# vvvvvw/Sentinel

Measured on AMD Instinct MI355X. Metric: decided entries/sec (whole node) at 1M resources; % of HBM roofline, higher is better.
Workload: dtype int64/f64

## Files before the change

sentinel_amd/csrc/engine.cpp:

```cpp
#include <hip/hip_runtime.h>

#include <algorithm>
#include <array>
#include <chrono>
#include <cmath>
#include <cstdint>
#include <cstdio>
#include <cstdlib>
#include <cstring>
#include <functional>
#include <map>
#include <set>
#include <string>
#include <unordered_map>
#include <vector>

#include "../../include/sentinel_gpu.h"
#include "authority.h"
#include "dev_types.h"
#include "pkeys.h"
#include "pmap.h"

namespace sg {
hipError_t launch_rs_first(const sg_event* ev, uint64_t n, uint32_t max_res, uint64_t gbase, const uint8_t* ring,
                           uint64_t ring_mask, int32_t max_rt, SEv* rec_o, uint32_t* keys, uint32_t* vals,
                           uint32_t* ghist, uint32_t nblocks, uint32_t* bflags, int64_t* t0_out, uint32_t* prio,
                           uint64_t* key_ring, const uint32_t* comp, const sg_event_ext* ext, const sg_arg* args,
                           uint64_t n_args, uint32_t max_ctx, const AuthDesc* auth, const uint32_t* auth_ids,
                           hipStream_t st);
hipError_t launch_radix_hist(const uint32_t* keys, uint64_t n, int shift, uint32_t* ghist, uint32_t nblocks,
                             hipStream_t st);
hipError_t launch_radix_hist_n(const uint32_t* keys, uint64_t n, const uint32_t* ndev, int shift, uint32_t* ghist,
                               uint32_t nblocks, hipStream_t st);
hipError_t launch_radix_scatter_n(const uint32_t* kin, const uint32_t* vin, uint64_t n, const uint32_t* ndev, int shift,
                                  const uint32_t* goff, uint32_t nblocks, uint32_t* kout, uint32_t* vout, hipStream_t st);
hipError_t launch_radix_scatter_x(const uint32_t* kin, const uint32_t* vin, uint64_t n, const uint32_t* ndev,
                                  const uint32_t* tcnt, const uint32_t* dbase, int shift, const uint32_t* goff,
                                  uint32_t nblocks, uint32_t* kout, uint32_t* vout, uint32_t* pos_of, hipStream_t st);
hipError_t launch_grp_first(const sg_event* ev, uint64_t n, uint32_t max_res, uint64_t gbase, uint64_t ring_mask,
                            uint32_t* bflags, int64_t* t0_out, uint32_t* prio, uint64_t* key_ring, const uint32_t* comp,
                            const sg_event_ext* ext, const sg_arg* args, uint64_t n_args, uint32_t max_ctx,
                            const AuthDesc* auth, const uint32_t* auth_ids,
                            const uint16_t* hot_tab, uint32_t nhot, uint32_t nblocks, uint32_t* words,
                            uint32_t* hot_hist, uint32_t* ckeys, uint32_t* cvals, uint32_t* ccnt, uint32_t* chist,
                            hipStream_t st);
hipError_t launch_hot_scan(uint32_t* C, uint32_t nblocks, uint32_t nhot, uint32_t* part, uint32_t* hb, uint32_t* total,
                           hipStream_t st);
hipError_t launch_hot_bmax(const sg_event* ev, uint32_t nblocks, const uint32_t* P, uint32_t nhot, const uint32_t* hb,
                           uint32_t* edges, uint32_t* bmax, hipStream_t st);
hipError_t launch_grp_records(const sg_event* ev, uint64_t n, uint64_t gbase, uint64_t ring_mask, int32_t max_rt,
                              const uint32_t* words, const uint32_t* P, uint32_t nhot, uint32_t nblocks,
                              const uint32_t* hb, SEv* recs, uint32_t* svals, uint32_t* prev,
                              uint32_t* nprev, uint32_t* bst, uint32_t* bflags, const sg_event_ext* ext,
                              const sg_arg* args, uint32_t max_ctx, Link* link, uint32_t epoch,
                              const uint32_t* need_hot, const uint32_t* need_blk, hipStream_t st);
hipError_t launch_hot_segs(const uint32_t* hb, uint32_t nhot, const uint32_t* hot_list, Seg* segs, uint32_t* out,
                           hipStream_t st);
hipError_t launch_hot_build(const Seg* segs, const uint32_t* mp, uint32_t mb, uint32_t min_len, uint32_t max_res, uint16_t* hot_tab,
                            uint32_t* hot_list, uint32_t nhot_old, uint32_t* hot_n, hipStream_t st);
hipError_t launch_cold_n(uint64_t n, const uint32_t* hot_total, uint32_t* out, hipStream_t st);
hipError_t launch_cold_small(const uint32_t* kin, const uint32_t* vin, const uint32_t* cnt, const uint32_t* dbase,
                             uint32_t* kout, uint32_t* vout, uint32_t* words, hipStream_t st);
uint32_t hot_max();
hipError_t launch_seg_cold(const uint32_t* keys, uint64_t n, const uint32_t* lo, const uint32_t* sbase, uint32_t* flag,
                           uint32_t* pos, Seg* segs, hipStream_t st,
                           hipError_t (*scan)(const uint32_t*, uint32_t*, uint64_t, uint32_t*, uint32_t*, hipStream_t),
                           uint32_t* part, uint32_t* ccount, uint32_t* nseg);
hipError_t launch_block_sums(const SEv* recs, uint64_t n, uint32_t* bst, Link* link, uint32_t epoch, uint32_t* bflags,
                             const uint32_t* skeys, const uint32_t* lo, const uint32_t* need_blk, hipStream_t st);
hipError_t launch_radix_scatter(const uint32_t* kin, const uint32_t* vin, uint64_t n, int shift, const uint32_t* goff,
                                uint32_t nblocks, uint32_t* kout, uint32_t* vout, uint32_t* pos_of, hipStream_t st);
uint32_t radix_tile();
hipError_t launch_scan(const uint32_t*, uint32_t*, uint64_t, uint32_t*, uint32_t*, hipStream_t);
hipError_t launch_snapshot(Bkt*, NodeInfo*, uint32_t, int64_t, int32_t, uint32_t*, uint32_t*, uint32_t*, uint32_t*,
                           sg_metric_node*, uint64_t, hipStream_t);
hipError_t launch_init_state(Bkt* sec, Bkt* minb, NodeInfo* info, int64_t* borrow, uint32_t nres, hipStream_t st);
hipError_t launch_set_flags(NodeInfo* info, const uint64_t* upd, uint32_t n, hipStream_t st);
hipError_t launch_region_copy(const uint64_t* src, uint64_t* dst, const uint64_t* tri, uint32_t n, hipStream_t st);
hipError_t launch_seg(const uint32_t* keys, uint64_t n, uint32_t* flag, uint32_t* pos, Seg* segs, hipStream_t st,
                      hipError_t (*scan)(const uint32_t*, uint32_t*, uint64_t, uint32_t*, uint32_t*, hipStream_t),
                      uint32_t* part, uint32_t* nseg);
hipError_t launch_seg_bin(Seg* segs, const uint32_t* mp, uint32_t mb, uint64_t n, const Prog* prog, const uint32_t* prio,
                          uint32_t lane_max, uint32_t j1_max, uint32_t j4_max, uint32_t force_lane, uint32_t* blkcnt,
                          uint32_t pq_ok, uint32_t pq_wide, uint32_t* aux, uint32_t* ashort, uint64_t* along,
                          uint64_t* amulti, uint32_t* mixc, uint32_t* mix, uint32_t mix_cap, uint32_t* mixlen,
                          uint32_t mix_wide, uint32_t head_min, const uint16_t* hot_tab, uint32_t nhot,
                          const uint32_t* nhotseg, uint32_t* need_hot, uint32_t* need_blk, const uint32_t* bmax,
                          uint32_t skip_min, uint32_t* nmark, hipStream_t st);
hipError_t launch_aux(const SEv* recs, const Seg* segs, const uint32_t* aux, const uint32_t* ashort,
                      const uint64_t* along, uint64_t* apiece, const uint64_t* amulti, const DevState& S, const DevCfg& cfg,
                      int64_t t0, const uint32_t* dec, AuxAcc* pool, uint32_t pool_cap, uint32_t* pool_n, uint64_t* meta,
                      uint32_t* bflags, hipStream_t st);
hipError_t launch_aux_cold(const SEv* recs, const Seg* segs, const uint32_t* aux, const uint32_t* ashort, const DevState& S,
                           const DevCfg& cfg, int64_t t0, const uint32_t* dec, uint32_t* bflags, hipStream_t st);
hipError_t launch_pq(int wide, const SEv* recs, const sg_event* ev, const uint32_t* vals, const Seg* segs,
                     const uint32_t* order, uint32_t m, const DevState& S, const DevCfg& cfg, int64_t t0, uint32_t* dec,
                     uint32_t* bflags, hipStream_t st);
hipError_t launch_pm_grow(const Seg* segs, const uint32_t* mp, uint32_t mb, const DevState& S, unsigned long long* pool_next,
                          uint64_t pool_nb, uint32_t* bflags, uint4* mv, uint32_t* nmv, uint32_t mcap, uint32_t epoch,
                          uint32_t nm, PBucket* b2, PData* d2, uint32_t* sz, uint32_t* off, uint32_t* part,
                          hipError_t (*scan)(const uint32_t*, uint32_t*, uint64_t, uint32_t*, uint32_t*, hipStream_t),
                          hipStream_t st);
hipError_t launch_pm_compact(PMap* pm, uint32_t n, const PBucket* ob, const PData* od, PBucket* nbk, PData* nd,
                             uint32_t* sz, uint32_t* off, uint32_t* part, unsigned long long* pool_next,
                             hipError_t (*scan)(const uint32_t*, uint32_t*, uint64_t, uint32_t*, uint32_t*, hipStream_t),
                             hipStream_t st);
hipError_t launch_pm_grow_ids(const uint32_t* ids, uint32_t n, const DevState& S, unsigned long long* pool_next,
                              uint64_t pool_nb, uint32_t* bflags, hipStream_t st);
hipError_t launch_pv_a(SEv* recs, const uint32_t* vals, Seg* segs, const uint32_t* list, uint32_t m,
                       const DevState& S, const DevCfg& cfg, uint32_t* dec, PvSeg* pv, PvBuf B, uint32_t cap,
                       uint32_t* tot, uint32_t* hist, uint32_t* part, hipStream_t st,
                       hipError_t (*radix_hist)(const uint32_t*, uint64_t, const uint32_t*, int, uint32_t*, uint32_t, hipStream_t),
                       hipError_t (*radix_scatter)(const uint32_t*, const uint32_t*, uint64_t, const uint32_t*, int,
                                                   const uint32_t*, uint32_t, uint32_t*, uint32_t*, hipStream_t),
                       hipError_t (*scan)(const uint32_t*, uint32_t*, uint64_t, uint32_t*, uint32_t*, hipStream_t),
                       uint32_t tile, uint32_t* rest, uint32_t grant_all);
hipError_t launch_pv_b(SEv* recs, Seg* segs, const uint32_t* list, uint32_t m, const DevState& S, int64_t t0,
                       uint32_t* dec, uint32_t* bflags, PvSeg* pv, PvBuf B, uint32_t cap, uint32_t* tot, uint32_t* part,
                       uint32_t jumps, hipStream_t st,
                       hipError_t (*scan)(const uint32_t*, uint32_t*, uint64_t, uint32_t*, uint32_t*, hipStream_t),
                       uint32_t* rest);
hipError_t launch_pvt(SEv* recs, const sg_event* ev, const uint32_t* vals, Seg* segs, const uint32_t* list, uint32_t m,
                      const DevState& S, const DevCfg& cfg, uint32_t* dec, uint32_t* bflags, PvSeg* pv, PvBuf B,
                      uint32_t cap, uint32_t* tot, uint32_t* hist, uint32_t* part, hipStream_t st,
                      hipError_t (*radix_hist)(const uint32_t*, uint64_t, const uint32_t*, int, uint32_t*, uint32_t, hipStream_t),
                      hipError_t (*radix_scatter)(const uint32_t*, const uint32_t*, uint64_t, const uint32_t*, int,
                                                      const uint32_t*, uint32_t, uint32_t*, uint32_t*, hipStream_t),
                      hipError_t (*scan)(const uint32_t*, uint32_t*, uint64_t, uint32_t*, uint32_t*, hipStream_t),
                      uint32_t tile, uint32_t* rest);
hipError_t launch_pq_mix(int post, SEv* recs, const sg_event* ev, const uint32_t* vals, const Seg* segs,
                         const uint32_t* list, uint32_t n_narrow, uint64_t wide_off, uint32_t n_wide, const DevState& S,
                         const DevCfg& cfg, int64_t t0, uint32_t* dec, uint32_t* bflags, hipStream_t st,
                         const uint32_t* rest, const uint32_t* rest_n);
hipError_t launch_seg_order(Seg* segs, const uint32_t* mp, uint32_t mb, const uint32_t* off, uint32_t* order,
                            uint32_t* bin_off, hipStream_t st);
hipError_t launch_gather(const SEv* rec_o, const uint32_t* vals, const uint32_t* skeys, uint64_t n,
                         const uint32_t* pos_of, SEv* recs, uint32_t* prev, uint32_t* nprev, Link* link, uint32_t* bst,
                         uint32_t epoch, uint32_t* bflags, hipStream_t st);
hipError_t launch_fill(const Span* spans, const uint32_t* nspan, uint32_t cap, const SEv* recs, const Prog* prog,
                       const DRule* rules, uint32_t* dec, hipStream_t st);
hipError_t launch_resolve(const uint32_t* prev, uint32_t np, const uint8_t* ring, SEv* recs, const uint32_t* vals,
                          const sg_event_ext* ext, hipStream_t st);
hipError_t launch_post_w(const uint32_t* words, const uint32_t* P, uint32_t nhot, const uint32_t* dec, uint64_t n,
                         uint64_t gbase, uint8_t* ring, uint64_t ring_mask, uint32_t* out, hipStream_t st);
hipError_t launch_post(const uint32_t* pos_of, const uint32_t* dec, uint64_t n, uint64_t gbase, uint8_t* ring,
                       uint64_t ring_mask, uint32_t* out, hipStream_t st);
hipError_t launch_chain(const SEv* recs, const uint32_t* vals, const Seg* segs, uint32_t m, NodeInfo* info,
                        uint32_t grant_all, uint32_t* ncand, uint64_t* cand, const sg_event* ev, const Prog* prog,
                        const sg_event_ext* ext, uint32_t max_ctx, hipStream_t st);
hipError_t launch_tiny(const sg_event* ev, uint32_t n, const DevState& S, const DevCfg& cfg, uint32_t max_res,
                       uint32_t* prio_w, const uint32_t* comp, uint64_t n_args, uint32_t grant_all,
                       unsigned long long* pool_next, uint64_t pool_nb, uint32_t epoch, SEv* recs, uint32_t* vals,
                       uint32_t* dec, Seg* segs, uint32_t* bflags, uint32_t* out, hipStream_t st);
uint32_t tiny_max();
hipError_t launch_decide_bin(int bin, const SEv* recs, const sg_event* ev, const uint32_t* vals, const Seg* segs,
                             const uint32_t* order, uint32_t m, const DevState& S, const DevCfg& cfg, int64_t t0,
                             uint32_t* dec, uint32_t* bflags, hipStream_t st);
hipError_t launch_tok_classify(const sg_token_req* req, uint64_t n, const CSlot* tab, uint32_t mask, uint32_t* fidx,
                               sg_token_result* res, uint32_t* flags, uint32_t* nskeys, uint32_t* nsvals, uint32_t nns,
                               hipStream_t st);
hipError_t launch_tok_limiter_ns(const sg_token_req* req, uint64_t n, const uint32_t* sk, const uint32_t* sv,
                                 const uint32_t* fidx, uint32_t nflows, NsLimiter* lims, const double* limits,
                                 uint32_t nns, uint32_t* keys, uint32_t* vals, sg_token_result* res, uint32_t* bflag,
                                 uint32_t* bidx, uint32_t* bstart, uint32_t* kpass, uint32_t* part, uint32_t* small,
                                 uint32_t* nsb,
                                 hipError_t (*scan)(const uint32_t*, uint32_t*, uint64_t, uint32_t*, uint32_t*, hipStream_t),
                                 hipStream_t st);
hipError_t launch_tok_limiter_par(const sg_token_req* req, uint64_t n, const uint32_t* fidx, uint32_t nflows,
                                  NsLimiter* lim, double allowed, uint32_t* keys, uint32_t* vals, sg_token_result* res,
                                  uint32_t* bflag, uint32_t* cflag, uint32_t* bidx, uint32_t* cexcl, uint32_t* bstart,
                                  uint32_t* kpass, uint32_t* part, uint32_t* small,
                                  hipError_t (*scan)(const uint32_t*, uint32_t*, uint64_t, uint32_t*, uint32_t*, hipStream_t),
                                  hipStream_t st);
hipError_t launch_tok_limiter(const sg_token_req* req, uint64_t n, const uint32_t* fidx, uint32_t nflows,
                              NsLimiter* lim, double allowed, uint32_t* keys, uint32_t* vals, sg_token_result* res,
                              hipStream_t st);
hipError_t launch_tok_flow(const uint32_t* skeys, const uint32_t* svals, uint64_t n, const sg_token_req* req,
                           CFlow* flows, uint32_t nflows, CBkt* bkts, double exceed, double max_occ_ratio,
                           sg_token_result* res, uint32_t* bounds, uint32_t light, uint32_t wide, hipStream_t st,
                           hipStream_t hs, hipEvent_t fork, hipEvent_t join);
hipError_t launch_ptok_flow(const uint32_t* skeys, const uint32_t* svals, uint64_t n, const sg_param_token_req* req,
                            const uint64_t* values, PFlow* flows, uint32_t nflows, const PHot* hot, PVal* tab,
                            uint32_t mask, sg_token_result* res, uint32_t* flags, hipStream_t st);
hipError_t launch_keysweep(const PMap* pmap, uint32_t nm, const PBucket* pbkt, uint64_t pool_nb, const uint64_t* pbm,
                           uint64_t bm_words, const uint64_t* key_ring, uint64_t ring_n, const PVal* pvtab,
                           uint64_t pv_n, const uint64_t* tkey, const uint32_t* tidx, uint32_t tmask, uint32_t* marks,
                           hipEvent_t* ev, hipStream_t st);
}

using namespace sg;

namespace {

thread_local std::string g_err;

int fail(int code, const std::string& msg) {
    g_err = msg;
    return code;
}

#define HIPCHK(x)                                                                                        \
    do {                                                                                                 \
        hipError_t _e = (x);                                                                             \
        if (_e != hipSuccess) return fail(SG_EDEVICE, std::string(#x ": ") + hipGetErrorString(_e));    \
    } while (0)

int32_t j_string_hash(const char* s) {
    if (!s) return 0;
    uint32_t h = 0;
    const unsigned char* p = (const unsigned char*)s;
    while (*p) {
        uint32_t cp;
        if (*p < 0x80) cp = *p++;
        else if ((*p & 0xE0) == 0xC0 && p[1]) { cp = ((p[0] & 0x1Fu) << 6) | (p[1] & 0x3Fu); p += 2; }
        else if ((*p & 0xF0) == 0xE0 && p[1] && p[2]) { cp = ((p[0] & 0x0Fu) << 12) | ((p[1] & 0x3Fu) << 6) | (p[2] & 0x3Fu); p += 3; }
        else if (p[1] && p[2] && p[3]) { cp = ((p[0] & 0x07u) << 18) | ((p[1] & 0x3Fu) << 12) | ((p[2] & 0x3Fu) << 6) | (p[3] & 0x3Fu); p += 4; }
// ... 168 lines not shown
              r.cluster_window_interval_ms % r.cluster_sample_count == 0))
            return false;
        if (r.cluster_flow_id <= 0) return false;
    }
    return true;
}
ParamR make_param(const sg_param_rule& s, const std::function<uint64_t(const char*, const char*)>& key) {
    ParamR p;
    p.r = s;
    p.res = sv(s.resource);
    p.la = la_norm(s.limit_app);
    for (int i = 0; i < s.n_items; ++i) {
        const sg_param_item& it = s.items[i];
        ParamItemR q;
        q.has_obj = it.object != nullptr;
        q.obj = sv(it.object);
        q.has_ct = it.class_type != nullptr;
        q.ct = sv(it.class_type);
        q.count = it.count;
        q.has_count = it.has_count;
        p.items.push_back(q);
        if (!it.object || !it.has_count || it.count < 0) continue;
        uint64_t k = key(it.object, it.class_type);
        bool found = false;
        for (auto& h : p.hot) if (h.first == k) { h.second = it.count; found = true; }
        if (!found) p.hot.push_back({k, it.count});
    }
    int32_t h = abstract_hash(s.resource, s.limit_app && !blank(s.limit_app) ? s.limit_app : "default");
    h = h31(h, s.grade);
    h = h31(h, s.has_param_idx ? s.param_idx : 0);
    h = h31(h, j_double_hash(s.count));
    h = h31(h, s.control_behavior);
    h = h31(h, s.max_queueing_time_ms);
    h = h31(h, s.burst_count);
    h = h31(h, long_hash(s.duration_in_sec));
    int32_t lh = 1;
    for (auto& q : p.items) {
        int32_t e = q.has_obj ? j_string_hash(q.obj.c_str()) : 0;
        e = h31(e, q.has_count ? q.count : 0);
        e = h31(e, q.has_ct ? j_string_hash(q.ct.c_str()) : 0);
        lh = h31(lh, e);
    }
    h = h31(h, lh);
    h = h31(h, s.cluster_mode ? 1 : 0);
    int32_t ch = 0;
    if (s.cluster_mode || s.cluster_flow_id)
        ch = cluster_hash(s.cluster_flow_id, s.cluster_threshold_type, s.cluster_fallback_to_local, 0,
                          s.cluster_sample_count, s.cluster_window_interval_ms, false);
    p.hash = h31(h, ch);
    char buf[512];
    std::snprintf(buf, sizeof(buf), "%d|%016llx|%d|%d|%d|%lld|%d|%d:%d|", s.grade, (unsigned long long)dbl_bits(s.count),
                  s.control_behavior, s.max_queueing_time_ms, s.burst_count, (long long)s.duration_in_sec,
                  s.cluster_mode ? 1 : 0, s.has_param_idx, s.has_param_idx ? s.param_idx : 0);
    std::string k = std::string(buf) + p.res + "\x01" + p.la + "\x01";
    for (auto& q : p.items) {
        std::snprintf(buf, sizeof(buf), "[%d%d%d:%d]", q.has_obj, q.has_ct, q.has_count, q.has_count ? q.count : 0);
        k += buf + q.obj + "\x02" + q.ct + "\x03";
    }
    if (s.cluster_mode || s.cluster_flow_id) {
        std::snprintf(buf, sizeof(buf), "C%lld|%d|%d|%d|%d", (long long)s.cluster_flow_id, s.cluster_threshold_type,
                      s.cluster_fallback_to_local ? 1 : 0, s.cluster_sample_count, s.cluster_window_interval_ms);
        k += buf;
    }
    p.eqkey = k;
    return p;
}

template <class T> void dfree(T*& p) {
    if (p) (void)hipFree(p);
    p = nullptr;
}

}

#define TMAP_KEY (1ull << 63)
struct sg_engine {
    sg_config cfg;
    int device = 0;
    hipStream_t stream = nullptr;
    double last_ms[4] = {0, 0, 0, 0};

    std::unordered_map<std::string, uint32_t> ids;
    std::vector<std::string> names;
    uint32_t n_chains = 0;

    bool flow_loaded = false, deg_loaded = false, par_loaded = false;
    std::vector<std::string> last_flow, last_deg, last_par;
    std::vector<FlowR> flows;
    std::vector<DegR> degs;
    std::vector<ParamR> params;
    std::vector<std::vector<int>> res_flow, res_deg, res_par;
    std::map<std::string, uint32_t> psid_of;
    uint32_t next_psid = 1;
    std::map<uint32_t, uint32_t> rmap_cap;
    std::set<uint64_t> tmaps;
    std::vector<uint64_t> pmap_key;
    std::unordered_map<uint32_t, uint32_t> pmap_index;
    std::vector<uint32_t> tm_base;
    uint64_t n_pslot = 0;
    uint64_t pool_nb = 0;
    unsigned long long* d_pool_next = nullptr;
    uint4* d_pmoves = nullptr;
    PBucket* d_pbkt2 = nullptr;
    PData* d_pdat2 = nullptr;
    uint32_t* d_pcwork = nullptr;
    uint64_t pmoves_cap = 0;
    unsigned long long* h_pool_next = nullptr;
    uint64_t n_compact = 0;
    uint64_t pool2_nb = 0;
    uint32_t n_dev_rules = 0;

    Bkt* d_sec = nullptr;
    Bkt* d_minb = nullptr;
    int64_t snap_hi = -1;
    NodeInfo* d_info = nullptr;
    Prog* d_prog = nullptr;
    DRule* d_rules = nullptr;
    RState* d_rstate = nullptr;
    DHot* d_hot = nullptr;
    PMap* d_pmap = nullptr;
    PBucket* d_pbkt = nullptr;
    PData* d_pdat = nullptr;
    uint64_t* d_pbm = nullptr;
    uint32_t* d_ppre = nullptr;
    uint32_t* d_tmid = nullptr;
    uint8_t* d_ring = nullptr;
    uint32_t rules_cap = 0, hot_cap = 0;

    struct BatchSlot {
        sg_event* d_ev = nullptr;
        uint32_t* d_out = nullptr;
        uint32_t *d_k0 = nullptr, *d_v0 = nullptr, *d_k1 = nullptr, *d_v1 = nullptr;
        uint32_t *d_hist = nullptr, *d_part = nullptr, *d_flag = nullptr, *d_pos = nullptr, *d_order = nullptr;
        uint32_t *d_posof = nullptr, *d_dec = nullptr, *d_blkcnt = nullptr, *d_prev = nullptr;
        SEv *d_recs = nullptr, *d_rec_o = nullptr;
        uint32_t* d_ccnt = nullptr;
        bool radix = false;
        uint32_t nhot = 0;
        uint32_t hot_marked = 0;
        Seg* d_segs = nullptr;
        uint64_t* d_cand = nullptr;
        uint32_t* d_bsmall = nullptr;
        sg_event_ext* d_ext = nullptr;
        sg_arg* d_args = nullptr;
        uint64_t ext_cap = 0, args_cap = 0;
        uint32_t* d_ashort = nullptr;
        uint64_t *d_apiece = nullptr, *d_amulti = nullptr, *d_along = nullptr;
        uint64_t aux_cap_n = 0;
        uint32_t* d_mix = nullptr;
        uint64_t mix_cap = 0;
        Link* d_link = nullptr;
        uint32_t *d_bst = nullptr, *d_pend = nullptr;
        Span* d_spans = nullptr;
        hipEvent_t ev[5] = {nullptr, nullptr, nullptr, nullptr, nullptr};
        bool pending = false;
    } slot[2];
    int cur = 0;
    int last = -1;
    hipStream_t gstream = nullptr;
    std::vector<std::array<double, 4>> tlog;
    std::string fatal;
    uint32_t* d_prio = nullptr;
    uint16_t* d_hot_tab = nullptr;
    uint32_t* d_hot_list = nullptr;
    uint32_t nhot = 0;
    uint32_t* d_hot_part = nullptr;
    uint32_t* d_hot_hb = nullptr;
    uint32_t* d_need = nullptr;
    uint64_t need_words = 0;
    uint32_t* d_edges = nullptr;
    uint32_t hot_marked_last = 0;
    bool radix_group = false;
    uint64_t radix_below = 1u << 18;
    uint32_t tok_light = 8192;
    uint32_t tok_wide = 1024;
    bool tiny_on = true;
    AuxNode* d_auxtab = nullptr;
    uint32_t* d_auxcnt = nullptr;
    uint64_t aux_mask = 0;
    AuxAcc* d_auxpool = nullptr;
    uint64_t* d_auxmeta = nullptr;
    uint32_t auxpool_cap = 0;
    uint64_t auxmeta_cap = 0;
    std::unordered_map<std::string, uint32_t> origin_ids, context_ids;
    std::unordered_map<std::string, int> rule_names;
    AuthTable auth;
    AuthDesc* d_auth = nullptr;
    uint32_t* d_auth_ids = nullptr;
    size_t auth_ids_cap = 0;
    bool auth_on = false, auth_loaded = false;
    std::vector<std::string> last_auth;
    uint32_t* d_comp = nullptr;
    uint32_t* d_prev = nullptr;
    uint32_t* d_bsmall = nullptr;
    Link* d_link = nullptr;
    uint32_t *d_bst = nullptr, *d_pend = nullptr;
    Span* d_spans = nullptr;
    uint32_t span_cap = 0;
    uint32_t epoch = 0;
    uint64_t spans_total = 0;
    uint64_t cap_n = 0;
    sg_event* d_ev = nullptr;
    uint32_t* d_out = nullptr;
    uint32_t *d_k0 = nullptr, *d_v0 = nullptr, *d_k1 = nullptr, *d_v1 = nullptr;
    uint32_t *d_hist = nullptr, *d_part = nullptr, *d_flag = nullptr, *d_pos = nullptr, *d_order = nullptr;
    uint32_t *d_posof = nullptr, *d_dec = nullptr, *d_blkcnt = nullptr;
    SEv *d_recs = nullptr, *d_rec_o = nullptr;
    Seg* d_segs = nullptr;
    uint32_t* d_small = nullptr;
    uint32_t* d_sink = nullptr;
    int64_t* d_borrow = nullptr;
    uint64_t* d_keyring = nullptr;
    uint64_t* d_cand = nullptr;
    uint32_t dbg_flags = 0;
    int prof_bin = 0;
    unsigned long long* d_dbg = nullptr;
    uint64_t cap_hist = 0;
    uint64_t gbase = 0;
    hipStream_t bin_stream[2] = {nullptr, nullptr};
    hipEvent_t fork = nullptr, join[2] = {nullptr, nullptr};
    hipEvent_t fork0 = nullptr;
    hipEvent_t grown = nullptr;
    bool pipeline = true;
    int j1_stream = -1;
    uint32_t lane_max = 256, j1_max = 4096, j4_max = 65536;
    uint32_t head_min = 0;
    bool bins_pinned = false;
    uint32_t skip_min = 32768;
    bool pq_on = true;
    uint32_t pq_wide = 8192;
    bool mix_on = true;
    bool mix_pq = false;
    bool pv_pq = true;
    bool has_mix = false;
    bool has_head = false;
    bool pv_on = true;
    PvBuf pvb{};
    PvBuf pvbt{};
    bool has_multi = false;
    uint64_t pv_cap = 0;
    PvSeg* d_pvseg = nullptr;
    PvSeg* d_pvtseg = nullptr;
    uint32_t* d_pvrest = nullptr;
    bool pvt_on = false;
    uint64_t pvseg_cap = 0;
    uint64_t pvch_cap = 0;
    uint32_t *d_pvtot = nullptr, *d_pvhist = nullptr, *d_pvpart = nullptr, *d_pvthist = nullptr, *d_pvtpart = nullptr;
    uint32_t pv_last_m = 0;
    bool skip_pinned = false;
    std::vector<CFlow> cflows;
    std::unordered_map<int64_t, uint32_t> cmap;
    CFlow* d_cflow = nullptr;
    CBkt* d_cbkt = nullptr;
    CSlot* d_ctab = nullptr;
    uint32_t ctab_mask = 0;
    uint64_t ncbkt = 0;
    NsLimiter* d_nslim = nullptr;
    std::vector<std::string> ns_names;
    std::unordered_map<std::string, uint32_t> ns_of;
    std::vector<double> ns_limit;
    std::vector<int32_t> ns_conn;
    std::unordered_map<int64_t, uint32_t> flow_ns;
    double* d_nslimit = nullptr;
    uint32_t* d_nsb = nullptr;
    bool tok_ns = false;
    sg_token_req* d_treq = nullptr;
    sg_token_result* d_tres = nullptr;
    uint32_t* d_tfidx = nullptr;
    uint32_t* d_tbounds = nullptr;
    uint32_t tbounds_cap = 0;
    uint64_t tcap = 0;
    std::vector<PFlow> pflows;
    std::unordered_map<int64_t, uint32_t> pmap;
    PFlow* d_pflow = nullptr;
    PHot* d_phot = nullptr;
    CSlot* d_pftab = nullptr;
    uint32_t pftab_mask = 0;
    PVal* d_pvtab = nullptr;
    uint32_t pv_mask = 0;
    sg_param_token_req* d_preq = nullptr;
    uint64_t* d_pvals = nullptr;
    uint64_t pcap = 0, pvcap = 0;
    pk::Dict<pk::StdHash> pkeys;
    std::vector<uint64_t> par_pins;
    uint64_t* d_ks_key = nullptr;
    uint32_t *d_ks_idx = nullptr, *d_ks_marks = nullptr;
    uint64_t ks_cap = 0;
    hipEvent_t ks_ev[4] = {nullptr, nullptr, nullptr, nullptr};
    uint64_t ks_sweeps = 0, ks_last[4] = {0, 0, 0, 0};
    double ks_scan_ms[3] = {0, 0, 0};
    uint64_t pbm_words = 0;
    uint32_t *d_snap_cnt = nullptr, *d_snap_off = nullptr;
    sg_metric_node* d_snap_out = nullptr;
    uint64_t snap_cap = 0;
};

namespace {

constexpr uint64_t SHARD_BATCH = 3ull << 21;

static void activate(sg_engine* e, int k) {
    auto& B = e->slot[k];
    e->d_ev = B.d_ev; e->d_out = B.d_out;
    e->d_k0 = B.d_k0; e->d_v0 = B.d_v0; e->d_k1 = B.d_k1; e->d_v1 = B.d_v1;
    e->d_hist = B.d_hist; e->d_part = B.d_part; e->d_flag = B.d_flag; e->d_pos = B.d_pos; e->d_order = B.d_order;
    e->d_posof = B.d_posof; e->d_dec = B.d_dec; e->d_blkcnt = B.d_blkcnt; e->d_prev = B.d_prev;
    e->d_recs = B.d_recs; e->d_rec_o = B.d_rec_o; e->d_segs = B.d_segs; e->d_cand = B.d_cand;
    e->d_bsmall = B.d_bsmall;
    e->d_link = B.d_link; e->d_bst = B.d_bst; e->d_pend = B.d_pend; e->d_spans = B.d_spans;
}
static void free_slot(sg_engine::BatchSlot& B) {
    dfree(B.d_ev); dfree(B.d_out); dfree(B.d_k0); dfree(B.d_v0); dfree(B.d_k1); dfree(B.d_v1);
    dfree(B.d_hist); dfree(B.d_part); dfree(B.d_flag); dfree(B.d_pos); dfree(B.d_order); dfree(B.d_segs);
    dfree(B.d_cand); dfree(B.d_posof); dfree(B.d_dec); dfree(B.d_recs); dfree(B.d_rec_o); dfree(B.d_blkcnt);
    dfree(B.d_prev); dfree(B.d_bsmall); dfree(B.d_ccnt);
    B.d_ccnt = nullptr;
    dfree(B.d_link); dfree(B.d_bst); dfree(B.d_pend); dfree(B.d_spans); dfree(B.d_ext); dfree(B.d_args);
    dfree(B.d_ashort); dfree(B.d_apiece); dfree(B.d_amulti); dfree(B.d_along); dfree(B.d_mix);
    B.d_mix = nullptr;
    B.ext_cap = B.args_cap = B.aux_cap_n = B.mix_cap = 0;
    B.d_link = nullptr; B.d_bst = B.d_pend = nullptr; B.d_spans = nullptr;
    B.d_ev = nullptr; B.d_out = nullptr; B.d_k0 = B.d_v0 = B.d_k1 = B.d_v1 = nullptr;
    B.d_hist = B.d_part = B.d_flag = B.d_pos = B.d_order = nullptr;
    B.d_posof = B.d_dec = B.d_blkcnt = B.d_prev = B.d_bsmall = nullptr;
    B.d_recs = B.d_rec_o = nullptr; B.d_segs = nullptr; B.d_cand = nullptr;
}
int ensure_batch(sg_engine* e, uint64_t n) {
    if (n <= e->cap_n) return SG_OK;
    uint64_t c = std::max<uint64_t>(n, 1u << 20);
    HIPCHK(hipStreamSynchronize(e->stream));
    uint64_t nblocks = (c + radix_tile() - 1) / radix_tile();
    e->cap_hist = nblocks * 256;
    for (auto& B : e->slot) {
        free_slot(B);
        HIPCHK(hipMalloc(&B.d_ev, c * sizeof(sg_event)));
        HIPCHK(hipMalloc(&B.d_out, c * 4));
        HIPCHK(hipMalloc(&B.d_k0, c * 4));
        HIPCHK(hipMalloc(&B.d_v0, c * 4));
        HIPCHK(hipMalloc(&B.d_k1, c * 4));
        HIPCHK(hipMalloc(&B.d_v1, c * 4));
        HIPCHK(hipMalloc(&B.d_hist, e->cap_hist * 4));
        HIPCHK(hipMalloc(&B.d_part, (e->cap_hist / 4096 + c / 4096 + 64) * 4));
        HIPCHK(hipMalloc(&B.d_flag, c * 4));
        HIPCHK(hipMalloc(&B.d_pos, c * 4));
        HIPCHK(hipMalloc(&B.d_order, c * 4));
        HIPCHK(hipMalloc(&B.d_segs, c * sizeof(Seg)));
        HIPCHK(hipMalloc(&B.d_cand, c * 8));
        HIPCHK(hipMalloc(&B.d_posof, c * 4));
        HIPCHK(hipMalloc(&B.d_dec, c * 4));
        HIPCHK(hipMalloc(&B.d_recs, c * sizeof(SEv)));
        const uint64_t co = (e->radix_group || c >= (1ull << 30)) ? c : std::min<uint64_t>(c, e->radix_below);
        if (co) HIPCHK(hipMalloc(&B.d_rec_o, co * sizeof(SEv)));
        HIPCHK(hipMalloc(&B.d_ccnt, 3 * (nblocks + 64) * 4));
    }
    dfree(e->d_hot_part);
    dfree(e->d_hot_hb);
    dfree(e->d_need);
    dfree(e->d_edges);
    e->need_words = hot_max() + c / 32768 + 2 + hot_max();
    HIPCHK(hipMalloc(&e->d_need, e->need_words * 4));
    HIPCHK(hipMalloc(&e->d_edges, (nblocks + 2) * 4));
    HIPCHK(hipMalloc(&e->d_hot_part, (nblocks / 16 + 2) * hot_max() * 4));
    HIPCHK(hipMalloc(&e->d_hot_hb, 2 * hot_max() * 4));
    for (auto& B : e->slot) {
        HIPCHK(hipMalloc(&B.d_blkcnt, ((c + 255) / 256 + 1) * N_BINS * 4));
        HIPCHK(hipMalloc(&B.d_prev, c * 4));
        HIPCHK(hipMalloc(&B.d_bsmall, 256 * 4));
        HIPCHK(hipMemset(B.d_bsmall, 0, 256 * 4));
        HIPCHK(hipMalloc(&B.d_link, c * sizeof(Link)));
        HIPCHK(hipMemset(B.d_link, 0, c * sizeof(Link)));
        HIPCHK(hipMalloc(&B.d_bst, ((c + 1023) / 1024 + 1) * 4));
        HIPCHK(hipMalloc(&B.d_pend, c * 4));
        HIPCHK(hipMalloc(&B.d_spans, (c / SPAN_CHUNK + 65536) * sizeof(Span)));
    }
    e->span_cap = (uint32_t)(c / SPAN_CHUNK + 65536);
    e->cap_n = c;
    activate(e, e->cur);
    return SG_OK;
}

static int collect(sg_engine* e, int k) {
    auto& B = e->slot[k];
    if (!B.pending) return SG_OK;
    B.pending = false;
    HIPCHK(hipEventSynchronize(B.ev[4]));
    float g = 0, d = 0, p = 0;
    (void)hipEventElapsedTime(&g, B.ev[0], B.ev[1]);
    (void)hipEventElapsedTime(&d, B.ev[2], B.ev[3]);
    (void)hipEventElapsedTime(&p, B.ev[3], B.ev[4]);
    (void)hipGetLastError();
    e->last_ms[0] = g; e->last_ms[1] = d; e->last_ms[2] = p; e->last_ms[3] = (double)g + d + p;
    e->tlog.push_back({(double)g, (double)d, (double)p, (double)g + d + p});
    if (e->tlog.size() > 4096) e->tlog.erase(e->tlog.begin(), e->tlog.begin() + 2048);
    uint32_t bflags = 0;
    HIPCHK(hipMemcpyAsync(&bflags, B.d_bsmall, 4, hipMemcpyDeviceToHost, e->gstream));
    uint32_t nspan = 0;
    HIPCHK(hipMemcpyAsync(&nspan, B.d_bsmall + 120, 4, hipMemcpyDeviceToHost, e->gstream));
    HIPCHK(hipStreamSynchronize(e->gstream));
    e->spans_total += nspan;
    e->hot_marked_last = B.hot_marked;
    if (bflags & BF_BAD_REF)
        return fail(SG_EINVAL, "an EXIT/TRACE references an event that is not an earlier ENTRY of the same resource");
    if (bflags & BF_BACKWARD)
        return fail(SG_EINVAL, "event timestamps must be non-decreasing across batches (SURVEY Q3)");
    if (bflags & BF_AUX_FULL) return fail(SG_ECAPACITY, "origin/context node pool full (raise aux_node_capacity)");
    if (bflags & BF_LITE_STALE)
        return fail(SG_ESTATE, "internal error (SG_LITE_CHECK): k_lite stored a minute bucket without a load that was not stale");
    if (bflags & BF_PQ_INVARIANT)
        e->fatal = "internal error: a k_pq tile's presorted key subset did not match its accesses";
    else if (bflags & BF_POOL_FULL)
        e->fatal = "the hot-parameter map pool is used up (raise param_table_log2)";
    else if (bflags & BF_PTAB_FULL)
        e->fatal = "a hot-parameter map table could not place a key (its map holds a ghost entry)";
    if (bflags & (BF_PQ_INVARIANT | BF_PTAB_FULL | BF_POOL_FULL)) return fail(SG_ECAPACITY, e->fatal + " -- engine unusable");
    return SG_OK;
}
static inline const AuthDesc* dev_auth(const sg_engine* e) { return e->auth_on ? e->d_auth : nullptr; }
static inline const uint32_t* dev_auth_ids(const sg_engine* e) { return e->auth_on ? e->d_auth_ids : nullptr; }

static int drain(sg_engine* e) {
    int rc = SG_OK;
    for (int i = 0; i < 2; ++i) {
        int r = collect(e, (e->cur + i) & 1);
        if (r && !rc) rc = r;
    }
    HIPCHK(hipStreamSynchronize(e->stream));
    return rc;
}


static uint32_t rule_map_cap(int64_t duration_sec) {
    const int64_t c = (int64_t)PM_BASE_CAP * std::max<int64_t>(duration_sec, 1);
    return (uint32_t)std::min<int64_t>(c, PM_TOTAL_CAP);
}

int upload_rules(sg_engine* e, bool reset_flow_state, bool reset_deg_state, bool reset_par_state) {
    uint32_t R = e->cfg.max_resources;
    std::vector<Prog> prog(R);
    std::vector<DRule> rules;
    std::vector<RState> rst;
    std::vector<DHot> hot;
    std::vector<RState> old_rst;
    std::vector<Prog> old_prog;
    if ((!reset_flow_state || !reset_deg_state || !reset_par_state) && e->n_dev_rules) {
        old_rst.resize(e->n_dev_rules);
        old_prog.resize(R);
        HIPCHK(hipMemcpy(old_rst.data(), e->d_rstate, e->n_dev_rules * sizeof(RState), hipMemcpyDeviceToHost));
        HIPCHK(hipMemcpy(old_prog.data(), e->d_prog, R * sizeof(Prog), hipMemcpyDeviceToHost));
    }
    size_t nres = e->names.size();
    bool any_mix = false, any_head = false;
    std::vector<std::pair<uint32_t, uint32_t>> relate;
    for (size_t r = 0; r < nres && r < R; ++r) {
        Prog p;
        std::memset(&p, 0, sizeof(p));
        p.rule_off = (uint32_t)rules.size();
        p.tm_base = r < e->tm_base.size() ? e->tm_base[r] : NO_ID;
        const auto& pl = r < e->res_par.size() ? e->res_par[r] : std::vector<int>();
        for (size_t i = 0; i < pl.size(); ++i) {
            const ParamR& q = e->params[pl[i]];
            DRule d;
            std::memset(&d, 0, sizeof(d));
            d.kind = RK_PARAM;
            d.grade = (uint8_t)q.r.grade;
            d.behavior = (uint8_t)q.r.control_behavior;
            if (q.r.cluster_mode && q.r.grade == SG_FLOW_GRADE_QPS && !q.r.cluster_fallback_to_local) {
                d.behavior = PB_INIT_ONLY;
                if (q.r.param_idx >= 0 && p.n_param && rules.back().behavior == PB_INIT_ONLY &&
                    rules.back().param_idx >= 0) {
                    if (q.r.param_idx < SG_MAX_ARGS) rules.back().burst |= (int32_t)(1u << q.r.param_idx);
                    continue;
                }
            }
            d.slot = (uint8_t)i;
            d.max_queue = q.r.max_queueing_time_ms;
            d.count = q.r.count;
            d.burst = q.r.burst_count;
            if (d.behavior == PB_INIT_ONLY && q.r.param_idx >= 0)
                d.burst = q.r.param_idx < SG_MAX_ARGS ? (int32_t)(1u << q.r.param_idx) : 0;
            double c = q.r.count;
            d.token_count = (c != c) ? 0 : c >= 2147483647.0 ? INT32_MAX : (int32_t)c;
            d.token_count_l = (c != c) ? 0 : c >= 9.2e18 ? INT64_MAX : (int64_t)c;
            d.duration_sec = q.r.duration_in_sec;
            d.hot_off = (uint32_t)hot.size();
            d.hot_n = (uint32_t)q.hot.size();
            for (auto& h : q.hot) hot.push_back(DHot{h.first, h.second, 0});
            d.pmap = e->pmap_index.at(e->psid_of.at(q.res + std::string("\0", 1) + q.eqkey));
            d.param_idx = q.r.param_idx;
            d.ref = NO_REF;
            rules.push_back(d);
            rst.push_back(RState{0, 0, 0, 0});
            p.n_param++;
        }
        const auto& fl = r < e->res_flow.size() ? e->res_flow[r] : std::vector<int>();
        std::vector<uint32_t> skipped_origins;
        for (size_t i = 0; i < fl.size(); ++i) {
            const FlowR& f = e->flows[fl[i]];
            if (!(f.r.cluster_mode && !f.r.cluster_fallback_to_local) || f.la == "default" || f.la == "other") continue;
            auto oi = e->origin_ids.find(f.la);
            if (oi != e->origin_ids.end()) skipped_origins.push_back(oi->second);
        }
        for (size_t i = 0; i < fl.size(); ++i) {
            const FlowR& f = e->flows[fl[i]];
            if (f.r.cluster_mode && !f.r.cluster_fallback_to_local) continue;
            DRule d;
            std::memset(&d, 0, sizeof(d));
            d.kind = RK_FLOW;
            d.grade = (uint8_t)f.r.grade;
            d.behavior = (uint8_t)(f.r.grade == SG_FLOW_GRADE_QPS ? f.r.control_behavior : SG_CONTROL_BEHAVIOR_DEFAULT);
            if (d.behavior > 3) d.behavior = SG_CONTROL_BEHAVIOR_DEFAULT;
            d.slot = (uint8_t)i;
            d.max_queue = f.r.max_queueing_time_ms;
            d.count = f.r.count;
            d.ref = NO_REF;
            d.la_kind = f.la == "default" ? LA_DEFAULT : f.la == "other" ? LA_OTHER : LA_ORIGIN;
            auto oi = e->origin_ids.find(f.la);
            d.la_origin = oi == e->origin_ids.end() ? NO_ID : oi->second;
            if (d.la_kind == LA_OTHER && !skipped_origins.empty()) {
                d.hot_off = (uint32_t)hot.size();
                d.hot_n = (uint32_t)skipped_origins.size();
                for (uint32_t o : skipped_origins) hot.push_back(DHot{o, 0, 0});
            }
            d.strategy = (uint32_t)f.r.strategy;
            d.chain_ctx = NO_ID;
            if (f.r.strategy == SG_STRATEGY_RELATE) {
                auto it = e->ids.find(f.ref);
                const uint32_t b = it == e->ids.end() ? NO_REF : it->second;
                if (b != NO_REF && b != (uint32_t)r && b < R) { d.ref = b; relate.emplace_back((uint32_t)r, b); }
            } else if (f.r.strategy == SG_STRATEGY_CHAIN) {
                if (f.ref == "sentinel_default_context") d.chain_ctx = 0;
                else {
                    auto ci = e->context_ids.find(f.ref);
                    if (ci != e->context_ids.end()) d.chain_ctx = ci->second;
                }
                p.multi |= PX_CHAIN;
            }
            if (d.la_kind != LA_DEFAULT && f.r.strategy == SG_STRATEGY_DIRECT) p.multi |= PX_ORIGIN;
            if (d.la_kind != LA_DEFAULT || f.r.strategy == SG_STRATEGY_CHAIN || f.r.strategy > SG_STRATEGY_CHAIN)
                p.pflags |= PF_SERIAL;
            if (d.behavior == SG_CONTROL_BEHAVIOR_WARM_UP || d.behavior == SG_CONTROL_BEHAVIOR_WARM_UP_RATE_LIMITER) {
                int cold = e->cfg.cold_factor;
                double c = f.r.count;
                auto d2i = [](double v) -> int32_t {
                    if (v != v) return 0;
                    if (v >= 2147483647.0) return INT32_MAX;
                    if (v <= -2147483648.0) return INT32_MIN;
                    return (int32_t)v;
                };
                int32_t wt = d2i(f.r.warm_up_period_sec * c) / (cold - 1);
                int32_t mt = (int32_t)((uint32_t)wt + (uint32_t)d2i((double)(2 * f.r.warm_up_period_sec) * c / (1.0 + cold)));
                d.warning_token = wt;
                d.max_token = mt;
                d.slope = (cold - 1.0) / c / (double)(mt - wt);
                d.count_div_cold = d2i(c) / cold;
                p.pflags |= PF_WARM;
            }
            rules.push_back(d);
            rst.push_back(RState{0, 0, -1, 0});
            p.n_flow++;
        }
        const auto& dl = r < e->res_deg.size() ? e->res_deg[r] : std::vector<int>();
        for (size_t i = 0; i < dl.size(); ++i) {
            const DegR& g = e->degs[dl[i]];
            DRule d;
            std::memset(&d, 0, sizeof(d));
            d.kind = RK_DEGRADE;
            d.grade = (uint8_t)g.r.grade;
            d.slot = (uint8_t)i;
            d.count = g.r.count;
            d.time_window = g.r.time_window;
            if (g.r.grade == SG_DEGRADE_GRADE_EXCEPTION_COUNT) p.pflags |= PF_EXC_COUNT;
            if (g.r.grade == SG_DEGRADE_GRADE_RT) p.pflags |= PF_RT;
            rules.push_back(d);
            rst.push_back(RState{0, 0, 0, 0});
            p.n_degrade++;
        }
        if ((int)p.n_param + p.n_flow + p.n_degrade > 16)
            return fail(SG_ENOTSUP, "more than 16 rules on one resource: " + e->names[r]);
        {
            int n_rl = 0;
// ... 84 lines not shown
        }
        for (uint32_t x = 0; x < R; ++x) comp[x] = find(x);
        std::vector<uint32_t> members;
        for (uint32_t x = 0; x < R; ++x)
            if (comp[x] != x) { members.push_back(x); members.push_back(comp[x]); }
        std::sort(members.begin(), members.end());
        members.erase(std::unique(members.begin(), members.end()), members.end());
        for (uint32_t x : members) {
            if (comp[x] == x) { prog[x].multi |= PX_MULTI; prog[x].pflags |= PF_SERIAL; }
        }
        any_multi = !members.empty();
        std::vector<NodeInfo> ni(members.size());
        for (size_t k = 0; k < members.size(); ++k)
            HIPCHK(hipMemcpy(&ni[k], e->d_info + members[k], sizeof(NodeInfo), hipMemcpyDeviceToHost));
        for (size_t k = 0; k < members.size(); ++k) {
            if (ni[k].flags & NI_CHAIN) ni[k].flags |= NI_TOUCHED;
            HIPCHK(hipMemcpy(e->d_info + members[k], &ni[k], sizeof(NodeInfo), hipMemcpyHostToDevice));
        }
        if (e->d_pmap) {
            const std::set<uint32_t> ms(members.begin(), members.end());
            std::vector<uint32_t> ids;
            for (uint32_t i = 0; i < (uint32_t)e->pmap_key.size(); ++i)
                if ((e->pmap_key[i] & TMAP_KEY) && ms.count((uint32_t)(e->pmap_key[i] >> 8))) ids.push_back(i);
            for (const auto& kv : e->psid_of) {
                auto it = e->ids.find(kv.first.substr(0, kv.first.find('\0')));
                auto pi = e->pmap_index.find(kv.second);
                if (it != e->ids.end() && ms.count(it->second) && pi != e->pmap_index.end()) ids.push_back(pi->second);
            }
            if (!ids.empty()) {
                uint32_t* d_ids = nullptr;
                HIPCHK(hipMalloc(&d_ids, ids.size() * 4));
                HIPCHK(hipMemcpy(d_ids, ids.data(), ids.size() * 4, hipMemcpyHostToDevice));
                DevState Sg{};
                std::memset(&Sg, 0, sizeof(Sg));
                Sg.pmap = e->d_pmap; Sg.pbkt = e->d_pbkt; Sg.pdat = e->d_pdat; Sg.pbm = e->d_pbm;
                HIPCHK(hipMemset(e->d_small, 0, 4));
                HIPCHK(launch_pm_grow_ids(d_ids, (uint32_t)ids.size(), Sg, e->d_pool_next, e->pool_nb, e->d_small, e->stream));
                uint32_t fl = 0;
                HIPCHK(hipMemcpyAsync(&fl, e->d_small, 4, hipMemcpyDeviceToHost, e->stream));
                HIPCHK(hipStreamSynchronize(e->stream));
                (void)hipFree(d_ids);
                if (fl & (BF_POOL_FULL | BF_PTAB_FULL))
                    return fail(SG_ECAPACITY, "hot-parameter map pool too small for the maps of STRATEGY_RELATE members "
                                              "(raise param_table_log2)");
            }
        }
    }
    if (rules.size() > e->cfg.max_rules) return fail(SG_ECAPACITY, "compiled rule table exceeds max_rules");
    if (rules.size() > e->rules_cap) {
        dfree(e->d_rules); dfree(e->d_rstate);
        e->rules_cap = (uint32_t)std::max<size_t>(rules.size(), 1024);
        HIPCHK(hipMalloc(&e->d_rules, e->rules_cap * sizeof(DRule)));
        HIPCHK(hipMalloc(&e->d_rstate, e->rules_cap * sizeof(RState)));
    }
    if (hot.size() > e->hot_cap) {
        dfree(e->d_hot);
        e->hot_cap = (uint32_t)std::max<size_t>(hot.size(), 1024);
        HIPCHK(hipMalloc(&e->d_hot, e->hot_cap * sizeof(DHot)));
    }
    HIPCHK(hipDeviceSynchronize());
    if (!rules.empty()) {
        HIPCHK(hipMemcpy(e->d_rules, rules.data(), rules.size() * sizeof(DRule), hipMemcpyHostToDevice));
        HIPCHK(hipMemcpy(e->d_rstate, rst.data(), rst.size() * sizeof(RState), hipMemcpyHostToDevice));
    }
    if (!hot.empty()) HIPCHK(hipMemcpy(e->d_hot, hot.data(), hot.size() * sizeof(DHot), hipMemcpyHostToDevice));
    HIPCHK(hipMemcpy(e->d_prog, prog.data(), R * sizeof(Prog), hipMemcpyHostToDevice));
    e->n_dev_rules = (uint32_t)rules.size();
    e->has_mix = any_mix;
    e->has_head = any_head;
    e->has_multi = any_multi;
    if (comp.empty()) {
        dfree(e->d_comp);
        e->d_comp = nullptr;
    } else {
        if (!e->d_comp) HIPCHK(hipMalloc(&e->d_comp, (uint64_t)R * 4));
        HIPCHK(hipMemcpy(e->d_comp, comp.data(), (uint64_t)R * 4, hipMemcpyHostToDevice));
    }
    return SG_OK;
}

uint32_t intern(sg_engine* e, const std::string& name) {
    auto it = e->ids.find(name);
    if (it != e->ids.end()) return it->second;
    uint32_t id = (uint32_t)e->names.size();
    e->ids.emplace(name, id);
    e->names.push_back(name);
    return id;
}

template <class V> void resize_lists(sg_engine* e, V& v) {
    if (v.size() < e->names.size()) v.resize(e->names.size());
}

}

extern "C" {

const char* sg_last_error(void) { return g_err.c_str(); }

void sg_config_default(sg_config* c) {
    std::memset(c, 0, sizeof(*c));
    c->sample_count = 2;
    c->interval_ms = 1000;
    c->statistic_max_rt = 4900;
    c->cold_factor = 3;
    c->occupy_timeout_ms = 500;
    c->max_slot_chain_size = 6000;
    c->switch_on = 1;
    c->device = 0;
    c->max_resources = 1u << 20;
    c->max_rules = 1u << 21;
    c->param_table_log2 = 28;
    c->status_ring_log2 = 28;
    c->max_batch_events = 1u << 25;
    c->cluster_sample_count = 10;
    c->cluster_interval_ms = 1000;
    c->cluster_exceed_count = 1.0;
    c->cluster_max_occupy_ratio = 1.0;
    c->cluster_max_allowed_qps = 30000;
    c->aux_node_capacity = 65536;
}

int sg_engine_create(const sg_config* cfg_in, sg_engine** out) {
    if (!out) return fail(SG_EINVAL, "out is null");
    sg_config cfg;
    if (cfg_in) cfg = *cfg_in;
    else sg_config_default(&cfg);
    if (cfg.sample_count != 2 || cfg.interval_ms != 1000)
        return fail(SG_ENOTSUP, "the device path implements SAMPLE_COUNT=2, INTERVAL=1000 (the reference defaults)");
    if (cfg.cold_factor <= 1) return fail(SG_EINVAL, "cold factor must be > 1");
    if (cfg.max_resources == 0 || cfg.param_table_log2 < 4 || cfg.param_table_log2 > 34 || cfg.status_ring_log2 < 10 ||
        cfg.status_ring_log2 > 36)
        return fail(SG_EINVAL, "bad capacity in sg_config");
    int ndev = 0;
    if (hipGetDeviceCount(&ndev) != hipSuccess || ndev == 0) return fail(SG_EDEVICE, "no HIP device visible");
    if (cfg.device < 0 || cfg.device >= ndev) return fail(SG_EDEVICE, "device ordinal out of range");
    hipDeviceProp_t prop;
    if (hipGetDeviceProperties(&prop, cfg.device) != hipSuccess) return fail(SG_EDEVICE, "hipGetDeviceProperties failed");
    if (std::strncmp(prop.gcnArchName, "gfx950", 6) != 0)
        return fail(SG_EDEVICE, std::string("this build targets gfx950, found ") + prop.gcnArchName);
    sg_engine* e = new sg_engine();
    e->cfg = cfg;
    e->device = cfg.device;
    auto bad = [&](int rc) { sg_engine_destroy(e); return rc; };
    if (hipSetDevice(e->device) != hipSuccess) return bad(fail(SG_EDEVICE, "hipSetDevice failed"));
    int prio_lo = 0, prio_hi = 0;
    const char* sp = std::getenv("SG_STREAM_PRIO");
    if (!(sp && sp[0] == '0')) (void)hipDeviceGetStreamPriorityRange(&prio_lo, &prio_hi);
    if (!(sp && sp[0] == '1')) std::swap(prio_lo, prio_hi);
    if (hipStreamCreateWithPriority(&e->stream, hipStreamNonBlocking, prio_hi) != hipSuccess) return bad(fail(SG_EDEVICE, "stream"));
    if (hipStreamCreateWithPriority(&e->gstream, hipStreamNonBlocking, prio_lo) != hipSuccess) {
        return bad(fail(SG_EDEVICE, "stream"));
    }
    for (auto& B : e->slot)
        for (auto& v : B.ev) if (hipEventCreate(&v) != hipSuccess) return bad(fail(SG_EDEVICE, "event"));
    uint64_t R = cfg.max_resources;
    if (hipMalloc(&e->d_sec, R * 2 * sizeof(Bkt)) != hipSuccess || hipMalloc(&e->d_minb, R * 60 * sizeof(Bkt)) != hipSuccess ||
        hipMalloc(&e->d_info, R * sizeof(NodeInfo)) != hipSuccess || hipMalloc(&e->d_prog, R * sizeof(Prog)) != hipSuccess ||
        hipMalloc(&e->d_ring, 1ull << cfg.status_ring_log2) != hipSuccess || hipMalloc(&e->d_small, 256 * 4) != hipSuccess ||
        hipMalloc(&e->d_sink, 1024 * 4) != hipSuccess || hipMalloc(&e->d_borrow, R * 4 * sizeof(int64_t)) != hipSuccess ||
        hipMalloc(&e->d_prio, R * 4) != hipSuccess || hipMalloc(&e->d_hot_tab, R * 2) != hipSuccess ||
        hipMalloc(&e->d_hot_list, hot_max() * 4) != hipSuccess)
        return bad(fail(SG_ENOMEM, "device allocation of the engine state failed"));
    {
        const uint64_t cap = std::max<uint32_t>(cfg.aux_node_capacity, 16u);
        uint64_t slots = 32;
        while (2 * slots < 3 * cap) slots <<= 1;
        e->aux_mask = slots - 1;
        e->cfg.aux_node_capacity = (uint32_t)cap;
        if (hipMalloc(&e->d_auxtab, slots * sizeof(AuxNode)) != hipSuccess || hipMalloc(&e->d_auxcnt, 4) != hipSuccess ||
            hipMemsetAsync(e->d_auxtab, 0xFF, slots * sizeof(AuxNode), e->stream) != hipSuccess ||
            hipMemsetAsync(e->d_auxcnt, 0, 4, e->stream) != hipSuccess)
            return bad(fail(SG_ENOMEM, "device allocation of the origin/context node table failed"));
    }
    if (hipMemsetAsync(e->d_prog, 0, R * sizeof(Prog), e->stream) != hipSuccess ||
        hipMemsetAsync(e->d_ring, 0xFF, 1ull << cfg.status_ring_log2, e->stream) != hipSuccess ||
        hipMemsetAsync(e->d_prio, 0, R * 4, e->stream) != hipSuccess ||
        hipMemsetAsync(e->d_hot_tab, 0xFF, R * 2, e->stream) != hipSuccess ||
        launch_init_state(e->d_sec, e->d_minb, e->d_info, e->d_borrow, (uint32_t)R, e->stream) != hipSuccess ||
        hipStreamSynchronize(e->stream) != hipSuccess)
        return bad(fail(SG_EDEVICE, "device initialisation failed"));
    for (auto& s : e->bin_stream)
        if (hipStreamCreateWithPriority(&s, hipStreamNonBlocking, prio_hi) != hipSuccess) return bad(fail(SG_EDEVICE, "stream"));
    if (hipEventCreateWithFlags(&e->fork, hipEventDisableTiming) != hipSuccess ||
        hipEventCreateWithFlags(&e->fork0, hipEventDisableTiming) != hipSuccess ||
        hipEventCreateWithFlags(&e->grown, hipEventDisableTiming) != hipSuccess)
        return bad(fail(SG_EDEVICE, "event"));
    for (auto& v : e->join)
        if (hipEventCreateWithFlags(&v, hipEventDisableTiming) != hipSuccess) return bad(fail(SG_EDEVICE, "event"));
    if (const char* d = std::getenv("SG_DEBUG")) {
        if (d[0] == '1' && hipMalloc(&e->d_dbg, 64 * 8) == hipSuccess) (void)hipMemset(e->d_dbg, 0, 64 * 8);
    }
    if (const char* f = std::getenv("SG_DEBUG_FLAGS")) e->dbg_flags = (uint32_t)std::strtoul(f, nullptr, 0);
    e->radix_group = (e->dbg_flags & 8192) != 0;
    if (const char* f = std::getenv("SG_PROF_BIN")) e->prof_bin = std::atoi(f);
    if (const char* v = std::getenv("SG_LANE_MAX")) { e->lane_max = (uint32_t)std::strtoul(v, nullptr, 0); e->bins_pinned = true; }
    if (const char* v = std::getenv("SG_J1_MAX")) { e->j1_max = (uint32_t)std::strtoul(v, nullptr, 0); e->bins_pinned = true; }
    if (const char* v = std::getenv("SG_HEAD_MIN")) e->head_min = (uint32_t)std::strtoul(v, nullptr, 0);
    if (const char* v = std::getenv("SG_J4_MAX")) { e->j4_max = (uint32_t)std::strtoul(v, nullptr, 0); e->bins_pinned = true; }
    if (const char* v = std::getenv("SG_PIPELINE")) e->pipeline = v[0] == '1';
    if (const char* v = std::getenv("SG_TINY")) e->tiny_on = v[0] != '0';
    if (const char* v = std::getenv("SG_LITE_CHECK")) { if (v[0] == '1') e->dbg_flags |= LITE_CHECK; }
    if (const char* v = std::getenv("SG_RADIX_BELOW")) e->radix_below = std::strtoull(v, nullptr, 0);
    if (const char* v = std::getenv("SG_TOK_WIDE")) e->tok_wide = std::atoi(v) == 512 ? 512u : 1024u;
    if (const char* v = std::getenv("SG_TOK_LIGHT")) e->tok_light = (uint32_t)std::strtoul(v, nullptr, 0);
    if (const char* v = std::getenv("SG_TOK_NS")) e->tok_ns = v[0] == '1';
    e->ns_names.push_back("default");
    e->ns_of["default"] = 0;
    e->ns_limit.push_back((double)cfg.cluster_max_allowed_qps);
    e->ns_conn.push_back(0);
    if (const char* v = std::getenv("SG_J1_STREAM")) e->j1_stream = std::atoi(v);
    if (const char* v = std::getenv("SG_PQ")) e->pq_on = v[0] != '0';
    if (const char* v = std::getenv("SG_MIX")) e->mix_on = v[0] != '0';
    if (const char* v = std::getenv("SG_MIX_PQ")) e->mix_pq = v[0] != '0';
    if (const char* v = std::getenv("SG_PV_PQ")) e->pv_pq = v[0] != '0';
    if (const char* v = std::getenv("SG_PV")) e->pv_on = v[0] != '0';
    e->pvt_on = e->pv_on;
    if (const char* v = std::getenv("SG_PVT")) e->pvt_on = v[0] != '0';
    if (const char* v = std::getenv("SG_PQ_WIDE")) e->pq_wide = (uint32_t)std::strtoul(v, nullptr, 0);
    if (const char* v = std::getenv("SG_SKIP_MIN")) {
        e->skip_min = std::max<uint32_t>(1u, (uint32_t)std::strtoul(v, nullptr, 0));
        e->skip_pinned = true;
    }
    *out = e;
    return SG_OK;
}

extern "C" int sgx_timing_log(sg_engine* e, double* out, int cap) {
    if (!e || !out) return 0;
    (void)drain(e);
    int k = 0;
    for (; k < cap && k < (int)e->tlog.size(); ++k)
        for (int j = 0; j < 4; ++j) out[4 * k + j] = e->tlog[k][j];
    e->tlog.clear();
    return k;
}
extern "C" unsigned long long sgx_spans_total(sg_engine* e) {
    if (!e) return 0;
    (void)drain(e);
    return e->spans_total;
}
extern "C" unsigned int sgx_hot_marked(sg_engine* e) {
    if (!e) return 0;
    (void)drain(e);
    return e->hot_marked_last;
}
extern "C" int sgx_debug_reset(sg_engine* e) {
    if (!e || !e->d_dbg) return 0;
    (void)drain(e);
    unsigned long long z[64] = {0};
    z[20] = ~0ull;
    return hipMemcpy(e->d_dbg, z, sizeof(z), hipMemcpyHostToDevice) == hipSuccess ? 1 : 0;
}
extern "C" int sgx_debug_counters(sg_engine* e, unsigned long long* out, int cap) {
    if (!e || !e->d_dbg || !out) return 0;
    int k = cap < 64 ? cap : 64;
    if (hipDeviceSynchronize() != hipSuccess) return 0;
    if (hipMemcpy(out, e->d_dbg, (size_t)k * 8, hipMemcpyDeviceToHost) != hipSuccess) return 0;
    return k;
}

extern "C" int sgx_read_aux_node(sg_engine* e, uint32_t res, uint32_t kind, uint32_t id, long long* out) {
    if (!e || !out || drain(e) != SG_OK) return -1;
    const unsigned long long key = ((unsigned long long)res << 32) | ((unsigned long long)kind << 31) | (id & 0x7FFFFFFFu);
    uint64_t h = mix64(key) & e->aux_mask;
    for (uint64_t probe = 0; probe <= e->aux_mask; ++probe) {
        AuxNode a;
        if (hipMemcpy(&a, e->d_auxtab + h, sizeof(a), hipMemcpyDeviceToHost) != hipSuccess) return -1;
        if (a.key == AUX_EMPTY) return 0;
        if (a.key == key) {
            for (int p = 0; p < 2; ++p) {
                const Bkt& b = a.sec[p];
                const int64_t v[8] = {b.ws, b.pass, b.block, b.exc, b.succ, b.rt, b.occ, b.minrt};
                for (int k = 0; k < 8; ++k) out[8 * p + k] = v[k];
            }
            out[16] = a.thread;
            out[17] = a.mws[0]; out[18] = a.mpass[0]; out[19] = a.mws[1]; out[20] = a.mpass[1];
            return 1;
        }
        h = (h + 1) & e->aux_mask;
    }
    return 0;
}
extern "C" int sgx_pv_last(sg_engine* e, unsigned long long* out) {
    if (!e || !out || drain(e) != SG_OK) return -1;
    out[0] = out[1] = out[2] = out[3] = out[4] = out[5] = out[6] = 0;
    if (!e->d_pvseg || !e->d_pvtot || !e->pv_last_m) return 0;
    std::vector<PvSeg> v(e->pv_last_m);
    uint32_t tot[8] = {0, 0, 0, 0, 0, 0, 0, 0};
    if (hipMemcpy(v.data(), e->d_pvseg, v.size() * sizeof(PvSeg), hipMemcpyDeviceToHost) != hipSuccess) return -1;
    if (hipMemcpy(tot, e->d_pvtot, 32, hipMemcpyDeviceToHost) != hipSuccess) return -1;
    for (const auto& s : v) out[0] += s.ok ? 1 : 0;
    out[1] = tot[0];
    out[2] = tot[2];
    out[6] = tot[3];
    if (e->pvt_on && e->d_pvtseg) {
        if (hipMemcpy(v.data(), e->d_pvtseg, v.size() * sizeof(PvSeg), hipMemcpyDeviceToHost) != hipSuccess) return -1;
        for (const auto& s : v) out[3] += s.ok ? 1 : 0;
        out[4] = tot[4];
        out[5] = tot[7];
    }
    if (!e->pv_on) out[0] = out[1] = out[2] = out[6] = 0;
    return 0;
}
extern "C" int sgx_param_pool(sg_engine* e, unsigned long long* out) {
    if (!e || !out || drain(e) != SG_OK) return -1;
    unsigned long long ctl[PC_WORDS] = {0, 0, 0, 0};
    if (e->d_pool_next && hipMemcpy(ctl, e->d_pool_next, sizeof(ctl), hipMemcpyDeviceToHost) != hipSuccess) return -1;
    out[0] = e->pool_nb; out[1] = ctl[PC_NEXT]; out[2] = ctl[PC_FLOOR]; out[3] = e->n_compact; out[4] = ctl[PC_RESCUES];
    return 0;
}

static int compact_pmaps(sg_engine* e);
extern "C" int sgx_param_compact(sg_engine* e) {
    if (!e || drain(e) != SG_OK) return -1;
    if (!e->pool_nb) return 0;
    if (compact_pmaps(e) != SG_OK) return -1;
    ++e->n_compact;
    return 0;
}

static void free_pv(sg_engine* e);

int sg_engine_destroy(sg_engine* e) {
    if (!e) return SG_OK;
    (void)hipSetDevice(e->device);
    if (e->stream) (void)hipStreamSynchronize(e->stream);
    if (e->gstream) (void)hipStreamSynchronize(e->gstream);
    dfree(e->d_sec); dfree(e->d_minb); dfree(e->d_info); dfree(e->d_prog); dfree(e->d_rules); dfree(e->d_rstate);
    dfree(e->d_hot); dfree(e->d_pmap); dfree(e->d_pbkt); dfree(e->d_pdat); dfree(e->d_pbm); dfree(e->d_ppre); dfree(e->d_tmid); dfree(e->d_ring); dfree(e->d_small); dfree(e->d_sink);
    dfree(e->d_pool_next); dfree(e->d_pmoves); dfree(e->d_pbkt2); dfree(e->d_pdat2); dfree(e->d_pcwork);
    if (e->h_pool_next) (void)hipHostFree(e->h_pool_next);
    free_pv(e);
    dfree(e->d_pvseg); dfree(e->d_pvtseg); dfree(e->d_pvtot); dfree(e->d_pvrest);
    if (e->gstream) (void)hipStreamSynchronize(e->gstream);
    for (auto& B : e->slot) free_slot(B);
    dfree(e->d_auth); dfree(e->d_auth_ids);
    dfree(e->d_prio); dfree(e->d_hot_tab); dfree(e->d_hot_list); dfree(e->d_hot_part); dfree(e->d_hot_hb); dfree(e->d_need); dfree(e->d_edges); dfree(e->d_comp); dfree(e->d_auxtab); dfree(e->d_auxpool); dfree(e->d_auxcnt); dfree(e->d_auxmeta);
    dfree(e->d_pflow); dfree(e->d_phot); dfree(e->d_pftab); dfree(e->d_pvtab); dfree(e->d_preq); dfree(e->d_pvals);
    dfree(e->d_cflow); dfree(e->d_cbkt); dfree(e->d_ctab); dfree(e->d_nslim); dfree(e->d_nslimit); dfree(e->d_nsb); dfree(e->d_borrow); dfree(e->d_keyring);
    dfree(e->d_treq); dfree(e->d_tres); dfree(e->d_tfidx); dfree(e->d_tbounds);
    dfree(e->d_snap_cnt); dfree(e->d_snap_off); dfree(e->d_snap_out); dfree(e->d_dbg);
    dfree(e->d_ks_key); dfree(e->d_ks_idx); dfree(e->d_ks_marks);
    for (auto& v : e->ks_ev) if (v) (void)hipEventDestroy(v);
    for (auto& B : e->slot)
        for (auto& v : B.ev) if (v) (void)hipEventDestroy(v);
    if (e->gstream) (void)hipStreamDestroy(e->gstream);
    for (auto& v : e->join) if (v) (void)hipEventDestroy(v);
    if (e->fork) (void)hipEventDestroy(e->fork);
    if (e->fork0) (void)hipEventDestroy(e->fork0);
    if (e->grown) (void)hipEventDestroy(e->grown);
    for (auto& s : e->bin_stream) if (s) (void)hipStreamDestroy(s);
    if (e->stream) (void)hipStreamDestroy(e->stream);
    delete e;
    return SG_OK;
}

int sg_register_resources(sg_engine* e, const char* const* names, uint32_t n, uint32_t* out_ids) {
    if (!e || (n && !names)) return fail(SG_EINVAL, "null argument");
    if (int rc = drain(e)) return rc;
    for (uint32_t i = 0; i < n; ++i) {
        if (!names[i]) return fail(SG_EINVAL, "null resource name");
        auto it = e->ids.find(names[i]);
        uint32_t id;
        if (it != e->ids.end()) id = it->second;
        else {
            if (e->names.size() >= e->cfg.max_resources) return fail(SG_ECAPACITY, "max_resources reached");
            id = intern(e, names[i]);
        }
        if (out_ids) out_ids[i] = id;
    }
    return SG_OK;
}

int sg_resource_id(sg_engine* e, const char* name, uint32_t* out_id) {
    if (!e || !name || !out_id) return fail(SG_EINVAL, "null argument");
    auto it = e->ids.find(name);
    if (it == e->ids.end()) return fail(SG_ENOTFOUND, std::string("unknown resource ") + name);
    *out_id = it->second;
    return SG_OK;
}

int sg_param_key(sg_engine* e, const char* value, const char* class_type, uint64_t* out_key) {
    (void)e;
    if (!out_key) return fail(SG_EINVAL, "null out_key");
    *out_key = param_key(value, class_type);
    return SG_OK;
}

static int register_rule_resource(sg_engine* e, const char* name, uint32_t* id) {
    auto it = e->ids.find(name);
    if (it != e->ids.end()) { *id = it->second; return SG_OK; }
    if (e->names.size() >= e->cfg.max_resources) return fail(SG_ECAPACITY, "max_resources reached");
    *id = intern(e, name);
    return SG_OK;
}

int sg_param_intern(sg_engine* e, const char* value, const char* class_type, uint64_t* out_key) {
    if (!e || !out_key) return fail(SG_EINVAL, "null argument");
    *out_key = e->pkeys.intern(value, class_type);
    return SG_OK;
}

int sg_param_intern_batch(sg_engine* e, const char* const* values, const char* const* class_types, uint32_t n,
                          uint64_t* out_keys) {
    if (!e || (n && (!values || !out_keys))) return fail(SG_EINVAL, "null argument");
    for (uint32_t i = 0; i < n; ++i) out_keys[i] = e->pkeys.intern(values[i], class_types ? class_types[i] : nullptr);
    return SG_OK;
}

int sg_param_keys_sweep(sg_engine* e) {
    if (!e) return fail(SG_EINVAL, "null engine");
    HIPCHK(hipSetDevice(e->device));
    if (int rc = drain(e)) return rc;
    const auto t_start = std::chrono::steady_clock::now();
    std::vector<uint64_t> cand;
    const uint64_t E = e->pkeys.sweep_begin(cand);
    const uint64_t nc = cand.size();
    std::vector<uint32_t> held((nc + 31) / 32, 0u);
    uint64_t n_held = 0;
    e->ks_scan_ms[0] = e->ks_scan_ms[1] = e->ks_scan_ms[2] = 0;
    const bool dev = (e->d_pmap && !e->pmap_key.empty()) || e->d_keyring || e->d_pvtab;
    if (nc && nc >= (1ull << 30)) return fail(SG_ECAPACITY, "too many sweep candidates for one table");
    if (nc && dev) {
        uint64_t slots = 16;
        while (slots < 2 * nc) slots <<= 1;
        if (slots > e->ks_cap) {
            dfree(e->d_ks_key); dfree(e->d_ks_idx); dfree(e->d_ks_marks);
            e->ks_cap = 0;
            HIPCHK(hipMalloc(&e->d_ks_key, slots * 8));
            HIPCHK(hipMalloc(&e->d_ks_idx, slots * 4));
            HIPCHK(hipMalloc(&e->d_ks_marks, ((slots + 31) / 32) * 4));
            e->ks_cap = slots;
        }
        for (auto& v : e->ks_ev)
            if (!v) HIPCHK(hipEventCreate(&v));
        std::vector<uint64_t> tk(slots, PK_EMPTY);
        std::vector<uint32_t> ti(slots, 0u);
        for (uint64_t i = 0; i < nc; ++i) {
            uint64_t h = (uint32_t)mix64(cand[i]) & (slots - 1);
            while (tk[h] != PK_EMPTY) h = (h + 1) & (slots - 1);
            tk[h] = cand[i];
            ti[h] = (uint32_t)i;
        }
        hipStream_t st = e->stream;
        HIPCHK(hipMemcpyAsync(e->d_ks_key, tk.data(), slots * 8, hipMemcpyHostToDevice, st));
        HIPCHK(hipMemcpyAsync(e->d_ks_idx, ti.data(), slots * 4, hipMemcpyHostToDevice, st));
        HIPCHK(hipMemsetAsync(e->d_ks_marks, 0, held.size() * 4, st));
        HIPCHK(launch_keysweep(e->pmap_key.empty() ? nullptr : e->d_pmap, (uint32_t)e->pmap_key.size(), e->d_pbkt,
                               e->pool_nb, e->d_pbm, e->pbm_words, e->d_keyring,
                               e->d_keyring ? 1ull << e->cfg.status_ring_log2 : 0, e->d_pvtab,
                               e->d_pvtab ? (uint64_t)e->pv_mask + 1 : 0, e->d_ks_key, e->d_ks_idx,
                               (uint32_t)(slots - 1), e->d_ks_marks, e->ks_ev, st));
        HIPCHK(hipMemcpyAsync(held.data(), e->d_ks_marks, held.size() * 4, hipMemcpyDeviceToHost, st));
        HIPCHK(hipStreamSynchronize(st));
        for (int k = 0; k < 3; ++k) {
            float ms = 0;
            if (hipEventElapsedTime(&ms, e->ks_ev[k], e->ks_ev[k + 1]) == hipSuccess) e->ks_scan_ms[k] = ms;
        }
        (void)hipGetLastError();
        for (uint32_t w : held) n_held += (uint64_t)__builtin_popcount(w);
    }
    const uint64_t dropped = e->pkeys.sweep_finish(E, cand, held.data());
    ++e->ks_sweeps;
    e->ks_last[0] = nc;
    e->ks_last[1] = n_held;
    e->ks_last[2] = dropped;
    e->ks_last[3] = (uint64_t)std::chrono::duration_cast<std::chrono::microseconds>(std::chrono::steady_clock::now() - t_start).count();
    return SG_OK;
}

int sg_param_keys_stats(sg_engine* e, uint64_t* out, int cap) {
    if (!e || !out) return 0;
    const pk::Stats s = e->pkeys.stats();
    const uint64_t v[8] = {s.entries, s.displaced, s.pinned, e->ks_sweeps, e->ks_last[0], e->ks_last[1], e->ks_last[2],
                           e->ks_last[3]};
    int k = 0;
    for (; k < cap && k < 8; ++k) out[k] = v[k];
    return k;
}
extern "C" int sgx_keysweep_scans(sg_engine* e, double* out) {
    if (!e || !out) return -1;
    for (int k = 0; k < 3; ++k) out[k] = e->ks_scan_ms[k];
    return 0;
}

static uint64_t tab_hash_h(int64_t k) {
    uint64_t z = (uint64_t)k + 0x9E3779B97F4A7C15ull;
    z = (z ^ (z >> 30)) * 0xBF58476D1CE4E5B9ull;
    z = (z ^ (z >> 27)) * 0x94D049BB133111EBull;
    return z ^ (z >> 31);
}
static uint32_t ns_index(const sg_engine* e, int64_t fid) {
    auto it = e->flow_ns.find(fid);
    return it == e->flow_ns.end() ? 0u : it->second;
}
static int rebuild_cluster(sg_engine* e, const sg_flow_rule* rules, uint32_t n) {
    std::vector<int64_t> order;
    std::unordered_map<int64_t, const sg_flow_rule*> rule_of;
// ... 590 lines not shown
        for (int i : per[r]) {
            const int32_t idx = ps[i].r.param_idx;
            for (int32_t k = 0; k < SG_MAX_ARGS; ++k)
                if (idx < 0 || idx == k) tmaps.insert(((uint64_t)r << 8) | (uint64_t)k);
        }
    uint64_t need = (rcap.size() + tmaps.size()) * (uint64_t)PM_MIN_NB * PM_BKT;
    if (need > (1ull << e->cfg.param_table_log2))
        return fail(SG_ECAPACITY, "hot-parameter maps need " + std::to_string(need) + " slots, param_table_log2 = " +
                                      std::to_string(e->cfg.param_table_log2) + " allows " +
                                      std::to_string(1ull << e->cfg.param_table_log2));
    if (int rc = rebuild_cluster_param(e, rules, all, n)) return rc;
    pins.end = 1;
    if (int rc = rebuild_pmaps(e, rcap, tmaps)) return rc;
    e->psid_of = std::move(psid_of);
    e->next_psid = next_psid;
    auto op = std::move(e->params);
    auto opr = std::move(e->res_par);
    e->params = std::move(ps);
    e->res_par = std::move(per);
    resize_lists(e, e->res_par);
    int rc = upload_rules(e, false, false, true);
    if (rc) { e->params = std::move(op); e->res_par = std::move(opr); return rc; }
    if (!clear_flags.empty()) {
        uint64_t* d = nullptr;
        HIPCHK(hipMalloc(&d, clear_flags.size() * 8));
        HIPCHK(hipMemcpy(d, clear_flags.data(), clear_flags.size() * 8, hipMemcpyHostToDevice));
        HIPCHK(launch_set_flags(e->d_info, d, (uint32_t)clear_flags.size(), e->stream));
        HIPCHK(hipStreamSynchronize(e->stream));
        (void)hipFree(d);
    }
    e->last_par = keys;
    e->par_loaded = true;
    pins.end = 2;
    if (!e->params.empty() && !e->d_keyring) {
        const uint64_t nk = 1ull << e->cfg.status_ring_log2;
        HIPCHK(hipMalloc(&e->d_keyring, nk * sizeof(uint64_t)));
        HIPCHK(hipMemset(e->d_keyring, 0xFF, nk * sizeof(uint64_t)));
    }
    if (n_loaded) *n_loaded = (uint32_t)e->params.size();
    return SG_OK;
}

static void free_pvbuf(PvBuf& B) {
    dfree(B.key); dfree(B.pos); dfree(B.dt); dfree(B.acq); dfree(B.tc); dfree(B.seg); dfree(B.gid); dfree(B.idx);
    dfree(B.gid2); dfree(B.idx2); dfree(B.prev); dfree(B.w); dfree(B.sprev); dfree(B.sw); dfree(B.fslot); dfree(B.hit);
    dfree(B.keep); dfree(B.flast); dfree(B.ftok); dfree(B.htab); dfree(B.chunk); dfree(B.ccnt); dfree(B.cof);
    dfree(B.gdt); dfree(B.gaw); dfree(B.gpos); dfree(B.range);
    B = PvBuf{};
}
static void free_pv(sg_engine* e) {
    free_pvbuf(e->pvb);
    free_pvbuf(e->pvbt);
    dfree(e->d_pvhist); dfree(e->d_pvpart); dfree(e->d_pvthist); dfree(e->d_pvtpart);
    e->d_pvhist = e->d_pvpart = e->d_pvthist = e->d_pvtpart = nullptr;
    e->pv_cap = 0;
    e->pvch_cap = 0;
}
static hipError_t drain_decide(sg_engine* e) {
    hipError_t r = hipStreamSynchronize(e->stream);
    for (auto s : e->bin_stream)
        if (r == hipSuccess && s) r = hipStreamSynchronize(s);
    return r;
}
static int ensure_pv(sg_engine* e, uint64_t cap, uint64_t m) {
    if (m > e->pvseg_cap) {
        HIPCHK(drain_decide(e));
        dfree(e->d_pvseg);
        dfree(e->d_pvtseg);
        e->pvseg_cap = std::max<uint64_t>(m + m / 2, 1024);
        HIPCHK(hipMalloc(&e->d_pvseg, e->pvseg_cap * sizeof(PvSeg)));
        HIPCHK(hipMalloc(&e->d_pvtseg, e->pvseg_cap * sizeof(PvSeg)));
        dfree(e->d_pvrest);
        HIPCHK(hipMalloc(&e->d_pvrest, 2 * (e->pvseg_cap + 1) * 4));
    }
    if (!e->d_pvtot) HIPCHK(hipMalloc(&e->d_pvtot, 64));
    if (cap > e->pv_cap) {
        HIPCHK(drain_decide(e));
        free_pv(e);
        const uint64_t c = std::max<uint64_t>(cap + cap / 4, 1u << 16);
        for (PvBuf* Bp : {&e->pvb, &e->pvbt}) {
            PvBuf& B = *Bp;
            HIPCHK(hipMalloc(&B.key, c * 8)); HIPCHK(hipMalloc(&B.pos, c * 4)); HIPCHK(hipMalloc(&B.dt, c * 4));
            HIPCHK(hipMalloc(&B.acq, c * 4)); HIPCHK(hipMalloc(&B.tc, c * 4)); HIPCHK(hipMalloc(&B.seg, c * 4));
            HIPCHK(hipMalloc(&B.gid, c * 4)); HIPCHK(hipMalloc(&B.idx, c * 4)); HIPCHK(hipMalloc(&B.gid2, c * 4));
            HIPCHK(hipMalloc(&B.idx2, c * 4)); HIPCHK(hipMalloc(&B.prev, c * 4)); HIPCHK(hipMalloc(&B.w, c * 4));
            HIPCHK(hipMalloc(&B.sprev, c * 4)); HIPCHK(hipMalloc(&B.sw, c * 4)); HIPCHK(hipMalloc(&B.fslot, c * 4));
            HIPCHK(hipMalloc(&B.hit, c)); HIPCHK(hipMalloc(&B.keep, c)); HIPCHK(hipMalloc(&B.flast, c * 8));
            HIPCHK(hipMalloc(&B.ftok, c * 4)); HIPCHK(hipMalloc(&B.htab, c * 16));
            HIPCHK(hipMalloc(&B.gdt, c * 4)); HIPCHK(hipMalloc(&B.gaw, c * 4)); HIPCHK(hipMalloc(&B.gpos, c * 4));
            HIPCHK(hipMalloc(&B.range, c * 16));
        }
        const uint64_t nblocks = (c + radix_tile() - 1) / radix_tile();
        HIPCHK(hipMalloc(&e->d_pvhist, nblocks * 256 * 4));
        HIPCHK(hipMalloc(&e->d_pvpart, nblocks * 256 * 4 + 4096));
        HIPCHK(hipMalloc(&e->d_pvthist, nblocks * 256 * 4));
        HIPCHK(hipMalloc(&e->d_pvtpart, nblocks * 256 * 4 + 4096));
        e->pv_cap = c;
    }
    const uint64_t nch = e->pv_cap / 4096 + m + 16;
    if (nch > e->pvch_cap) {
        HIPCHK(drain_decide(e));
        e->pvch_cap = nch + nch / 2;
        for (PvBuf* Bp : {&e->pvb, &e->pvbt}) {
            PvBuf& B = *Bp;
            dfree(B.chunk); dfree(B.ccnt); dfree(B.cof);
            HIPCHK(hipMalloc(&B.chunk, e->pvch_cap * 8)); HIPCHK(hipMalloc(&B.ccnt, e->pvch_cap * 4));
            HIPCHK(hipMalloc(&B.cof, e->pvch_cap * 4 + 4));
        }
    }
    return SG_OK;
}

static int ensure_mix(sg_engine::BatchSlot& B, uint64_t mb) {
    if (mb > B.mix_cap) {
        dfree(B.d_mix);
        B.mix_cap = std::max<uint64_t>(mb, 1u << 12);
        HIPCHK(hipMalloc(&B.d_mix, B.mix_cap * 2 * 4));
    }
    return SG_OK;
}

#define AUXPOOL_CAP (1u << 20)
static int ensure_aux(sg_engine* e, sg_engine::BatchSlot& B, uint64_t n) {
    const uint64_t npiece = n / AUX_PIECE + n / 257 + 64;
    if (n > B.aux_cap_n) {
        dfree(B.d_ashort); dfree(B.d_apiece); dfree(B.d_amulti); dfree(B.d_along);
        const uint64_t c = std::max<uint64_t>(n, 1u << 16);
        HIPCHK(hipMalloc(&B.d_ashort, c * 4));
        HIPCHK(hipMalloc(&B.d_along, (c / 257 + 64) * 8));
        HIPCHK(hipMalloc(&B.d_apiece, (c / AUX_PIECE + c / 257 + 64) * 8));
        HIPCHK(hipMalloc(&B.d_amulti, (c / AUX_PIECE + 64) * 8));
        B.aux_cap_n = c;
    }
    if (!e->d_auxpool) {
        HIPCHK(hipMalloc(&e->d_auxpool, (uint64_t)AUXPOOL_CAP * sizeof(AuxAcc)));
        e->auxpool_cap = AUXPOOL_CAP;
    }
    if (npiece > e->auxmeta_cap) {
        HIPCHK(hipStreamSynchronize(e->stream));
        dfree(e->d_auxmeta);
        const uint64_t c = std::max<uint64_t>(npiece, B.aux_cap_n / AUX_PIECE + B.aux_cap_n / 257 + 64);
        HIPCHK(hipMalloc(&e->d_auxmeta, c * 8));
        e->auxmeta_cap = c;
    }
    return SG_OK;
}

static bool is_device_ptr(const void* p) {
    hipPointerAttribute_t a;
    if (hipPointerGetAttributes(&a, p) != hipSuccess) { (void)hipGetLastError(); return false; }
    return a.type == hipMemoryTypeDevice || a.type == hipMemoryTypeManaged;
}

static int submit_impl(sg_engine* e, const sg_event* ev, const sg_event_ext* ext, uint64_t n, const sg_arg* args,
                       uint64_t n_args, uint32_t* out) {
    if (!e || (n && (!ev || !out))) return fail(SG_EINVAL, "null argument");
    if (n_args && !args) return fail(SG_EINVAL, "null args table");
    if (!e->fatal.empty()) return fail(SG_ESTATE, e->fatal + " -- engine unusable, recreate it");
    if (n == 0) return SG_OK;
    if (n > e->cfg.max_batch_events || n >= (1ull << 31)) return fail(SG_EINVAL, "batch larger than max_batch_events");
    HIPCHK(hipSetDevice(e->device));
    int rc = ensure_batch(e, n);
    if (rc) return rc;
    const int k = e->cur;
    rc = collect(e, k);
    if (rc) return rc;
    if (int prc = ensure_pool2(e)) return prc;
    const unsigned long long pfloor = e->h_pool_next ? e->h_pool_next[PC_FLOOR] : 0;
    if (e->pool_nb && e->h_pool_next[PC_NEXT] > pfloor + (e->pool_nb - pfloor) / 2) {
        if (int drc = drain(e)) return drc;
        if (int crc = compact_pmaps(e)) return crc;
        ++e->n_compact;
    }
    activate(e, k);
    auto& B = e->slot[k];
    hipStream_t gs = e->gstream, st = e->stream;
    const sg_event* dev_ev = ev;
    bool host_in = !is_device_ptr(ev);
    bool host_out = !is_device_ptr(out);
    if (host_in) {
        HIPCHK(hipMemcpyAsync(e->d_ev, ev, n * sizeof(sg_event), hipMemcpyHostToDevice, gs));
        dev_ev = e->d_ev;
    }
    uint32_t* dev_out = host_out ? e->d_out : out;
    const sg_event_ext* dev_ext = ext;
    const sg_arg* dev_args = n_args ? args : nullptr;
    if (ext && !is_device_ptr(ext)) {
        if (n > B.ext_cap) {
            dfree(B.d_ext);
            B.ext_cap = std::max<uint64_t>(n, 1u << 16);
            HIPCHK(hipMalloc(&B.d_ext, B.ext_cap * sizeof(sg_event_ext)));
        }
        HIPCHK(hipMemcpyAsync(B.d_ext, ext, n * sizeof(sg_event_ext), hipMemcpyHostToDevice, gs));
        dev_ext = B.d_ext;
    }
    if (n_args && !is_device_ptr(args)) {
        if (n_args > B.args_cap) {
            dfree(B.d_args);
            B.args_cap = std::max<uint64_t>(n_args, 1u << 16);
            HIPCHK(hipMalloc(&B.d_args, B.args_cap * sizeof(sg_arg)));
        }
        HIPCHK(hipMemcpyAsync(B.d_args, args, n_args * sizeof(sg_arg), hipMemcpyHostToDevice, gs));
        dev_args = B.d_args;
    }
    const uint64_t ring_mask = (1ull << e->cfg.status_ring_log2) - 1;
    if (!e->pipeline && e->last >= 0 && e->slot[e->last].pending)
        HIPCHK(hipStreamWaitEvent(gs, e->slot[e->last].ev[4], 0));
    HIPCHK(hipEventRecord(B.ev[0], gs));
    uint32_t R = e->cfg.max_resources;
    int bits = 1;
    while (bits < 32 && (1ull << bits) < R) ++bits;
    const int db = 8;
    int passes = (bits + db - 1) / db;
    uint32_t nblocks = (uint32_t)((n + radix_tile() - 1) / radix_tile());
    HIPCHK(hipMemsetAsync(e->d_bsmall, 0, 256 * 4, gs));
    int64_t* d_t0 = reinterpret_cast<int64_t*>(e->d_bsmall + 4);
    uint32_t *kin = e->d_k1, *vin = e->d_v1, *kout = e->d_k0, *vout = e->d_v0;
    if (++e->epoch == 0) e->epoch = 1;
    B.radix = e->radix_group || n >= (1ull << 30) || n < e->radix_below;
    const bool force_lane = !e->cfg.switch_on || (e->dbg_flags & 2);
    const uint32_t mb = (uint32_t)std::min<uint64_t>(n, R);
    const uint32_t nblk = (mb + 255) / 256;
    uint32_t lane_max = e->lane_max, j1_max = e->j1_max, j4_max = e->j4_max;
    if (!e->bins_pinned && n < SHARD_BATCH) {
        lane_max = std::min<uint32_t>(lane_max, 128);
        j1_max = std::min<uint32_t>(j1_max, 1024);
        j4_max = std::min<uint32_t>(j4_max, 4096);
    }
    j1_max = std::min<uint32_t>(j1_max, 64u * 65000u);
    j4_max = std::min<uint32_t>(j4_max, 256u * 65000u);
    const uint32_t skip_min = (!e->skip_pinned && n < SHARD_BATCH) ? std::min<uint32_t>(e->skip_min, 8192) : e->skip_min;
    auto bins = [&](uint32_t* need_hot, uint32_t* need_blk, const uint32_t* bmax) -> int {
        if (ext) {
            if (int arc = ensure_aux(e, B, n)) return arc;
        }
        if (e->has_mix) {
            if (int mrc = ensure_mix(B, mb)) return mrc;
        }
        HIPCHK(launch_seg_bin(e->d_segs, e->d_bsmall + 1, mb, n, e->d_prog, e->d_prio, lane_max, j1_max, j4_max,
                              force_lane ? 1 : 0, e->d_blkcnt, e->pq_on ? 1u : 0u, e->pq_wide, ext ? e->d_bsmall + 130 : nullptr,
                              B.d_ashort, B.d_along, B.d_amulti, e->d_bsmall + 6, e->has_mix ? B.d_mix : nullptr,
                              (uint32_t)B.mix_cap, e->d_bsmall + 72, (e->pv_on || e->pvt_on) ? 0u : e->pq_wide,
                              (e->dbg_flags & HEAD_OFF) ? 0u : e->head_min, e->d_hot_tab, e->nhot, e->d_bsmall + 80, need_hot,
                              need_blk, bmax, skip_min, e->d_bsmall + 73, gs));
        HIPCHK(launch_scan(e->d_blkcnt, e->d_blkcnt, (uint64_t)nblk * N_BINS, e->d_part, nullptr, gs));
        HIPCHK(launch_seg_order(e->d_segs, e->d_bsmall + 1, mb, e->d_blkcnt, e->d_order, e->d_bsmall + 8, gs));
        return SG_OK;
    };
    if (B.radix) {
        HIPCHK(launch_rs_first(dev_ev, n, R, e->gbase, e->d_ring, ring_mask, e->cfg.statistic_max_rt, e->d_rec_o,
                               e->d_k1, e->d_v1, e->d_hist, nblocks, e->d_bsmall + 0, d_t0, e->d_prio, e->d_keyring,
                               e->d_comp, dev_ext, dev_args, n_args, SG_MAX_CONTEXTS, dev_auth(e), dev_auth_ids(e), gs));
        for (int p = 0; p < passes; ++p) {
            if (p > 0) HIPCHK(launch_radix_hist(kin, n, p * db, e->d_hist, nblocks, gs));
            HIPCHK(launch_scan(e->d_hist, e->d_hist, (uint64_t)nblocks << db, e->d_part, nullptr, gs));
            HIPCHK(launch_radix_scatter(kin, vin, n, p * db, e->d_hist, nblocks, kout, vout,
                                        p == passes - 1 ? e->d_posof : nullptr, gs));
            std::swap(kin, kout);
            std::swap(vin, vout);
        }
        HIPCHK(launch_seg(kin, n, e->d_flag, e->d_pos, e->d_segs, gs, launch_scan, e->d_part, e->d_bsmall + 1));
        HIPCHK(launch_gather(e->d_rec_o, vin, kin, n, e->d_posof, e->d_recs, e->d_prev, e->d_bsmall + 3, e->d_link,
                             e->d_bst, e->epoch, e->d_bsmall + 0, gs));
        if (int brc = bins(nullptr, nullptr, nullptr)) return brc;
    } else {
        const uint32_t nhot = e->nhot;
        B.nhot = nhot;
        uint32_t* words = e->d_flag;
        uint32_t* hot_off = e->d_pos;
        uint32_t* ccnt = B.d_ccnt;
        HIPCHK(launch_grp_first(dev_ev, n, R, e->gbase, ring_mask, e->d_bsmall + 0, d_t0, e->d_prio, e->d_keyring,
                                e->d_comp, dev_ext, dev_args, n_args, SG_MAX_CONTEXTS, dev_auth(e), dev_auth_ids(e),
                                e->d_hot_tab, nhot, nblocks,
                                words, hot_off, e->d_k1, e->d_v1, ccnt, e->d_hist, gs));
        HIPCHK(launch_hot_scan(hot_off, nblocks, nhot, e->d_hot_part, e->d_hot_hb, e->d_bsmall + 77, gs));
        HIPCHK(launch_cold_n(n, e->d_bsmall + 77, e->d_bsmall + 78, gs));
        if (nblocks == 1) {
            HIPCHK(launch_cold_small(kin, vin, ccnt, e->d_bsmall + 77, kout, vout, words, gs));
            std::swap(kin, kout);
            std::swap(vin, vout);
        }
        for (int p = 0; p < passes && nblocks > 1; ++p) {
            if (p > 0) HIPCHK(launch_radix_hist_n(kin, n, e->d_bsmall + 78, p * db, e->d_hist, nblocks, gs));
            HIPCHK(launch_scan(e->d_hist, e->d_hist, (uint64_t)nblocks << db, e->d_part, nullptr, gs));
            const bool last = p == passes - 1;
            HIPCHK(launch_radix_scatter_x(kin, vin, n, p ? e->d_bsmall + 78 : nullptr, p ? nullptr : ccnt,
                                          last ? e->d_bsmall + 77 : nullptr, p * db, e->d_hist, nblocks, kout, vout,
                                          last ? words : nullptr, gs));
            std::swap(kin, kout);
            std::swap(vin, vout);
        }
        HIPCHK(launch_hot_segs(e->d_hot_hb, nhot, e->d_hot_list, e->d_segs, e->d_bsmall + 80, gs));
        const uint64_t sc = nblocks + 64;
        HIPCHK(launch_seg_cold(kin, n, e->d_bsmall + 77, e->d_bsmall + 80, ccnt + sc, ccnt + 2 * sc, e->d_segs, gs,
                               launch_scan, e->d_part, e->d_bsmall + 82, e->d_bsmall + 1));
        HIPCHK(hipMemsetAsync(e->d_bst, 0, ((n + 1023) / 1024) * 4, gs));
        uint32_t *need_hot = nullptr, *need_blk = nullptr, *bmax = nullptr;
        if (!(e->dbg_flags & TABLES_ALL)) {
            need_hot = e->d_need;
            need_blk = e->d_need + hot_max();
            bmax = e->d_need + e->need_words - hot_max();
            HIPCHK(hipMemsetAsync(e->d_need, 0, e->need_words * 4, gs));
            HIPCHK(launch_hot_bmax(dev_ev, nblocks, hot_off, nhot, e->d_hot_hb, e->d_edges, bmax, gs));
        }
        if (int brc = bins(need_hot, need_blk, bmax)) return brc;
        HIPCHK(launch_grp_records(dev_ev, n, e->gbase, ring_mask, e->cfg.statistic_max_rt, words, hot_off, nhot, nblocks,
                                  e->d_hot_hb, e->d_recs, vin, e->d_prev, e->d_bsmall + 3, e->d_bst,
                                  e->d_bsmall + 0, dev_ext, dev_args, SG_MAX_CONTEXTS, e->d_link, e->epoch, need_hot,
                                  need_blk, gs));
        HIPCHK(launch_block_sums(e->d_recs, n, e->d_bst, e->d_link, e->epoch, e->d_bsmall + 0, kin, e->d_bsmall + 77,
                                 need_blk, gs));
    }
    const uint32_t hot_min = (uint32_t)std::max<uint64_t>(64, n / 8192);
    if (!B.radix)
        HIPCHK(launch_hot_build(e->d_segs, e->d_bsmall + 1, mb, hot_min, R, e->d_hot_tab, e->d_hot_list, e->nhot,
                                e->d_bsmall + 76, gs));
    uint32_t head[77];
    static_assert(8 + N_BINS + 1 <= 72, "head layout");
    HIPCHK(hipMemcpyAsync(head, e->d_bsmall, sizeof(head), hipMemcpyDeviceToHost, gs));
    HIPCHK(hipEventRecord(B.ev[1], gs));
    HIPCHK(hipStreamSynchronize(gs));
    if (!B.radix) e->nhot = std::min<uint32_t>(head[76], hot_max());
    B.hot_marked = head[73];
    const uint32_t m = head[1];
    const uint32_t nprev = head[3];
    int64_t t0 = 0;
    std::memcpy(&t0, head + 4, 8);
    uint32_t bflags = head[0];
    if (bflags & BF_BAD_RES) return fail(SG_EINVAL, "event res_id >= max_resources");
    if (bflags & BF_BAD_REF)
        return fail(SG_EINVAL, "an EXIT/TRACE references an event that is not an earlier ENTRY of the same resource");
    if (bflags & BF_TSPAN) return fail(SG_EINVAL, "a batch must span less than 2^31 ms");
    if (bflags & BF_BACKWARD) return fail(SG_EINVAL, "event timestamps must be non-decreasing (SURVEY Q3)");
    if (bflags & BF_BAD_ARGS)
        return fail(SG_EINVAL, "an sg_event_ext names args outside the table (or more than SG_MAX_ARGS, or a bad kind)");
    const uint32_t* off = head + 8;
    uint32_t bin_n[N_BINS];
    for (int b = 0; b < N_BINS; ++b) bin_n[b] = off[b + 1] - off[b];
    DevCfg dc;
    std::memset(&dc, 0, sizeof(dc));
    dc.max_rt = e->cfg.statistic_max_rt;
    dc.occupy_timeout = e->cfg.occupy_timeout_ms;
    dc.max_chain = e->cfg.max_slot_chain_size;
    dc.switch_on = e->cfg.switch_on;
    dc.ring_mask = ring_mask;
    dc.snap_hi = e->snap_hi;
    dc.dbg_flags = e->dbg_flags;
    dc.heads = e->has_head ? 1u : 0u;
    DevState S{};
    std::memset(&S, 0, sizeof(S));
    S.sec = e->d_sec;
    S.minb = e->d_minb;
    S.info = e->d_info;
    S.prog = e->d_prog;
    S.rules = e->d_rules;
    S.rstate = e->d_rstate;
    S.hot = e->d_hot;
    S.pmap = e->d_pmap;
    S.pbkt = e->d_pbkt;
    S.pdat = e->d_pdat;
    S.pbm = e->d_pbm;
    S.ppre = e->d_ppre;
    S.tmid = e->d_tmid;
    S.ring = e->d_ring;
    S.sink = e->d_sink;
    S.borrow = e->d_borrow;
    S.prio = e->d_prio;
    S.key_ring = e->d_keyring;
    S.gbase = e->gbase;
    S.link = e->d_link;
    S.bst = e->d_bst;
    S.pend = e->d_pend;
    S.spans = e->d_spans;
    S.nspan = e->d_bsmall + 120;
    S.span_cap = e->span_cap;
    S.epoch = e->epoch;
    S.skip_ok = !(bflags & (BF_MULTI_LINK | BF_ZERO_CNT)) && !(e->dbg_flags & 4) ? 1u : 0u;
    S.skip_min = skip_min;
    S.ext = dev_ext;
    S.args = dev_args;
    S.aux_tab = e->d_auxtab;
    S.aux_count = e->d_auxcnt;
    S.aux_cap = e->cfg.aux_node_capacity;
    S.aux_mask = e->aux_mask;
    S.max_ctx = SG_MAX_CONTEXTS;
    S.auth = dev_auth(e);
    S.auth_ids = dev_auth_ids(e);
    HIPCHK(hipStreamWaitEvent(st, B.ev[1], 0));
    const uint32_t n_mix = e->has_mix ? head[6] : 0u, n_mixw = e->has_mix ? head[7] : 0u;
    const bool serial_bins = (e->dbg_flags & 8) != 0;
    const bool pre_split = (n_mix || n_mixw) && !serial_bins;
    hipStream_t ps = pre_split ? e->bin_stream[1] : st;
    const uint32_t grant_all = (e->cfg.switch_on && e->cfg.max_slot_chain_size <= 0) ? 1u : 0u;
    if (n_mixw && (e->pv_on || e->pvt_on) && head[72]) {
        if (int prc = ensure_pv(e, head[72], n_mixw)) return prc;
        e->pv_last_m = n_mixw;
    }
    const bool pv_ran = n_mixw && e->pv_on && head[72];
    const bool pv_early = pv_ran && pre_split && grant_all && !e->has_multi;
    if (pv_early) {
        HIPCHK(hipStreamWaitEvent(ps, B.ev[1], 0));
        HIPCHK(launch_pv_a(e->d_recs, vin, e->d_segs, B.d_mix + B.mix_cap, n_mixw, S, dc, e->d_dec, e->d_pvseg, e->pvb,
                           head[72], e->d_pvtot, e->d_pvhist, e->d_pvpart, ps, launch_radix_hist_n,
                           launch_radix_scatter_n, launch_scan, radix_tile(), e->d_pvrest, grant_all));
    }
    HIPCHK(launch_resolve(e->d_prev, nprev, e->d_ring, e->d_recs, vin, dev_ext, st));
    if (e->cfg.switch_on && (e->cfg.max_slot_chain_size <= 0 || e->n_chains < (uint32_t)e->cfg.max_slot_chain_size)) {
        const bool grant_all = e->cfg.max_slot_chain_size <= 0;
        HIPCHK(launch_chain(e->d_recs, vin, e->d_segs, m, e->d_info, grant_all ? 1 : 0, e->d_bsmall + 2, e->d_cand,
                            dev_ev, e->d_prog, dev_ext, SG_MAX_CONTEXTS, st));
        if (!grant_all) {
            uint32_t ncand = 0;
            HIPCHK(hipMemcpyAsync(&ncand, e->d_bsmall + 2, 4, hipMemcpyDeviceToHost, st));
            HIPCHK(hipStreamSynchronize(st));
            if (ncand) {
                std::vector<uint64_t> cand(ncand);
                HIPCHK(hipMemcpy(cand.data(), e->d_cand, ncand * 8ull, hipMemcpyDeviceToHost));
                std::sort(cand.begin(), cand.end());
                std::vector<uint64_t> upd;
                std::unordered_map<uint32_t, int> seen;
                for (uint32_t i = 0; i < ncand; ++i) {
                    uint32_t res = (uint32_t)cand[i];
                    if (!seen.emplace(res, 1).second) continue;
                    bool grant = e->n_chains < (uint32_t)e->cfg.max_slot_chain_size;
                    if (grant) e->n_chains++;
                    upd.push_back(((uint64_t)(grant ? NI_CHAIN : NI_REJECTED) << 32) | res | (1ull << 63));
                }
                ncand = (uint32_t)upd.size();
                HIPCHK(hipMemcpyAsync(e->d_cand, upd.data(), ncand * 8ull, hipMemcpyHostToDevice, st));
                HIPCHK(launch_set_flags(e->d_info, e->d_cand, ncand, st));
                HIPCHK(hipStreamSynchronize(st));
            }
        }
    }
    if (pre_split) {
        HIPCHK(hipEventRecord(e->fork0, st));
        HIPCHK(hipStreamWaitEvent(ps, e->fork0, 0));
    }
    if (pv_ran && !pv_early)
        HIPCHK(launch_pv_a(e->d_recs, vin, e->d_segs, B.d_mix + B.mix_cap, n_mixw, S, dc, e->d_dec, e->d_pvseg, e->pvb,
                           head[72], e->d_pvtot, e->d_pvhist, e->d_pvpart, ps, launch_radix_hist_n,
                           launch_radix_scatter_n, launch_scan, radix_tile(), e->d_pvrest, grant_all));
    if (e->pool_nb) {
        DevState Sg{};
        std::memset(&Sg, 0, sizeof(Sg));
        Sg.prog = e->d_prog; Sg.rules = e->d_rules; Sg.tmid = e->d_tmid; Sg.prio = e->d_prio;
        Sg.pmap = e->d_pmap; Sg.pbkt = e->d_pbkt; Sg.pdat = e->d_pdat; Sg.pbm = e->d_pbm;
        const uint32_t nm = (uint32_t)e->pmap_key.size();
        HIPCHK(launch_pm_grow(e->d_segs, e->d_bsmall + 1, mb, Sg, e->d_pool_next, e->pool_nb, e->d_bsmall + 0, e->d_pmoves,
                              e->d_pmoves ? reinterpret_cast<uint32_t*>(e->d_pmoves + e->pmoves_cap) : nullptr,
                              (uint32_t)e->pmoves_cap, e->epoch, nm, e->d_pbkt2, e->d_pdat2, e->d_pcwork,
                              e->d_pcwork + e->pmoves_cap, e->d_pcwork + 2 * e->pmoves_cap, launch_scan, st));
        HIPCHK(hipMemcpyAsync(e->h_pool_next, e->d_pool_next, PC_WORDS * 8, hipMemcpyDeviceToHost, st));
    }
    HIPCHK(hipEventRecord(B.ev[2], st));
    if (pre_split) {
        HIPCHK(hipEventRecord(e->grown, st));
        HIPCHK(hipStreamWaitEvent(ps, e->grown, 0));
    }
    if (pv_ran) {
        HIPCHK(launch_pv_b(e->d_recs, e->d_segs, B.d_mix + B.mix_cap, n_mixw, S, t0, e->d_dec, e->d_bsmall + 0,
                           e->d_pvseg, e->pvb, head[72], e->d_pvtot, e->d_pvpart, (bflags & BF_ZERO_CNT) ? 0u : 1u, ps,
                           launch_scan, e->d_pvrest));
    }
    if (n_mix || n_mixw)
        HIPCHK(launch_pq_mix(0, e->d_recs, dev_ev, vin, e->d_segs, B.d_mix, n_mix, B.mix_cap, n_mixw, S, dc, t0,
                             e->d_dec, e->d_bsmall + 0, ps, pv_ran ? e->d_pvrest + 1 : nullptr, e->d_pvrest));
    HIPCHK(hipEventRecord(e->fork, ps));
    auto lane_bins = [&]() -> int {
        {
            DevState Sl = S;
            Sl.dbg = e->d_dbg;
            HIPCHK(launch_decide_bin(BIN_LANE, e->d_recs, dev_ev, vin, e->d_segs, e->d_order + off[BIN_LANE],
                                     off[BIN_LANE + LANE_BINS] - off[BIN_LANE], Sl, dc, t0, e->d_dec, e->d_bsmall + 0, st));
        }
        HIPCHK(launch_decide_bin(BIN_LANE16, e->d_recs, dev_ev, vin, e->d_segs, e->d_order + off[BIN_LANE16],
                                 off[BIN_LANE16 + LANE_BINS] - off[BIN_LANE16], S, dc, t0, e->d_dec, e->d_bsmall + 0, st));
        {
            DevState Sl = S;
            Sl.dbg = e->d_dbg;
            HIPCHK(launch_decide_bin(BIN_LITE, e->d_recs, dev_ev, vin, e->d_segs, e->d_order + off[BIN_LITE],
                                     off[BIN_LITE + LANE_BINS] - off[BIN_LITE], Sl, dc, t0, e->d_dec, e->d_bsmall + 0, st));
        }
        return SG_OK;
    };
    if (pre_split) {
        if (int lrc = lane_bins()) return lrc;
        HIPCHK(hipStreamWaitEvent(st, e->fork, 0));
    }
    const int coop[2] = {BIN_J16, BIN_J4};
    const bool j8_own = bin_n[BIN_J8] && !bin_n[BIN_J16];
    for (int c = 0; c < 2; ++c) {
        const int b = coop[c];
        if (c == 0 && bin_n[BIN_J8]) {
            DevState Sb = S;
            Sb.dbg = (e->prof_bin == 0 && e->d_dbg) ? e->d_dbg : nullptr;
            hipStream_t bs = (serial_bins || !j8_own) ? st : e->bin_stream[0];
            if (bs != st) HIPCHK(hipStreamWaitEvent(bs, e->fork, 0));
            HIPCHK(launch_decide_bin(BIN_J8, e->d_recs, dev_ev, vin, e->d_segs, e->d_order + off[BIN_J8], bin_n[BIN_J8], Sb, dc,
                                     t0, e->d_dec, e->d_bsmall + 0, bs));
            if (bs != st) HIPCHK(hipEventRecord(e->join[0], bs));
        }
        if (!bin_n[b]) continue;
        DevState Sb = S;
        Sb.dbg = (c == e->prof_bin && e->d_dbg) ? e->d_dbg : nullptr;
        hipStream_t bs = serial_bins ? st : e->bin_stream[c];
        if (!serial_bins) HIPCHK(hipStreamWaitEvent(bs, e->fork, 0));
        HIPCHK(launch_decide_bin(b, e->d_recs, dev_ev, vin, e->d_segs, e->d_order + off[b], bin_n[b], Sb, dc, t0,
                                 e->d_dec, e->d_bsmall + 0, bs));
        HIPCHK(hipEventRecord(e->join[c], bs));
    }
    for (int c = 0; c < 2; ++c) {
        const int b = c == 0 ? BIN_PQ16 : BIN_PQ4;
        if (!bin_n[b]) continue;
        hipStream_t bs = serial_bins ? st : e->bin_stream[c];
        if (!serial_bins && !bin_n[coop[c]] && !(c == 0 && j8_own)) HIPCHK(hipStreamWaitEvent(bs, e->fork, 0));
        DevState Sp = S;
        Sp.dbg = (c == 0 && e->prof_bin == 3) ? e->d_dbg : nullptr;
        HIPCHK(launch_pq(c == 0, e->d_recs, dev_ev, vin, e->d_segs, e->d_order + off[b], bin_n[b], Sp, dc, t0, e->d_dec,
                         e->d_bsmall + 0, bs));
        HIPCHK(hipEventRecord(e->join[c], bs));
    }
    if (!pre_split)
        if (int lrc = lane_bins()) return lrc;
    const bool aux_early = ext && !bin_n[BIN_PQ4] && !serial_bins && (force_lane || lane_max >= 256u) &&
                           (!bin_n[BIN_PQ16] || e->pq_wide >= 256u);
    if (aux_early)
        HIPCHK(launch_aux_cold(e->d_recs, e->d_segs, e->d_bsmall + 130, B.d_ashort, S, dc, t0, e->d_dec, e->d_bsmall + 0, st));
    const bool j1_b0 = bin_n[BIN_J1] && !serial_bins && (e->j1_stream == 1 || (e->j1_stream < 0 && aux_early));
    const bool j1_split = bin_n[BIN_J1] > 1 && !serial_bins && e->j1_stream == 2;
    if (j1_split) {
        const uint32_t h = bin_n[BIN_J1] / 2;
        for (int c = 0; c < 2; ++c) {
            DevState Sj = S;
            Sj.dbg = nullptr;
            hipStream_t bs = e->bin_stream[c];
            const bool ran = c == 0 ? (bin_n[BIN_J16] || bin_n[BIN_J8] || bin_n[BIN_PQ16]) : (bin_n[BIN_J4] || bin_n[BIN_PQ4]);
            if (!ran) HIPCHK(hipStreamWaitEvent(bs, e->fork, 0));
            HIPCHK(launch_decide_bin(BIN_J1, e->d_recs, dev_ev, vin, e->d_segs, e->d_order + off[BIN_J1] + (c ? h : 0),
                                     c ? bin_n[BIN_J1] - h : h, Sj, dc, t0, e->d_dec, e->d_bsmall + 0, bs));
            HIPCHK(hipEventRecord(e->join[c], bs));
        }
    } else if (bin_n[BIN_J1]) {
        DevState Sj = S;
        Sj.dbg = (e->prof_bin == 2 && e->d_dbg) ? e->d_dbg : nullptr;
        hipStream_t bs = j1_b0 ? e->bin_stream[0] : st;
        if (j1_b0 && !(bin_n[BIN_J16] || bin_n[BIN_J8] || bin_n[BIN_PQ16])) HIPCHK(hipStreamWaitEvent(bs, e->fork, 0));
        HIPCHK(launch_decide_bin(BIN_J1, e->d_recs, dev_ev, vin, e->d_segs, e->d_order + off[BIN_J1], bin_n[BIN_J1], Sj, dc,
                                 t0, e->d_dec, e->d_bsmall + 0, bs));
        if (j1_b0) HIPCHK(hipEventRecord(e->join[0], bs));
    }
    for (int c = 0; c < 2; ++c)
        if (bin_n[coop[c]] || bin_n[c == 0 ? BIN_PQ16 : BIN_PQ4] || (c == 0 && (j8_own || j1_b0)) || j1_split)
            HIPCHK(hipStreamWaitEvent(st, e->join[c], 0));
    if (S.skip_ok && (bin_n[BIN_J16] || bin_n[BIN_J8] || bin_n[BIN_J4]))
        HIPCHK(launch_fill(e->d_spans, S.nspan, e->span_cap, e->d_recs, e->d_prog, e->d_rules, e->d_dec, st));
    if (n_mixw && e->pvt_on && head[72])
        HIPCHK(launch_pvt(e->d_recs, dev_ev, vin, e->d_segs, B.d_mix + B.mix_cap, n_mixw, S, dc, e->d_dec,
                          e->d_bsmall + 0, e->d_pvtseg, e->pvbt, head[72], e->d_pvtot + 4, e->d_pvthist, e->d_pvtpart, st,
                          launch_radix_hist_n, launch_radix_scatter_n, launch_scan, radix_tile(),
                          e->d_pvrest + e->pvseg_cap + 1));
    const bool pvt_ran = n_mixw && e->pvt_on && head[72];
    uint32_t* prest = e->d_pvrest + e->pvseg_cap + 1;
    if (n_mix || n_mixw)
        HIPCHK(launch_pq_mix(1, e->d_recs, dev_ev, vin, e->d_segs, B.d_mix, n_mix, B.mix_cap, n_mixw, S, dc, t0,
                             e->d_dec, e->d_bsmall + 0, st, pvt_ran ? prest + 1 : nullptr, prest));
    if (ext)
        HIPCHK(launch_aux(e->d_recs, e->d_segs, e->d_bsmall + 130, aux_early ? nullptr : B.d_ashort, B.d_along, B.d_apiece,
                          B.d_amulti, S, dc, t0, e->d_dec, e->d_auxpool, e->auxpool_cap, e->d_bsmall + 134, e->d_auxmeta,
                          e->d_bsmall + 0, st));
    HIPCHK(hipEventRecord(B.ev[3], st));
    if (B.radix) HIPCHK(launch_post(e->d_posof, e->d_dec, n, e->gbase, e->d_ring, ring_mask, dev_out, st));
    else HIPCHK(launch_post_w(e->d_flag, e->d_pos, B.nhot, e->d_dec, n, e->gbase, e->d_ring, ring_mask, dev_out, st));
    if (host_out) HIPCHK(hipMemcpyAsync(out, dev_out, n * 4, hipMemcpyDeviceToHost, st));
    HIPCHK(hipEventRecord(B.ev[4], st));
    B.pending = true;
    e->last = k;
    e->cur = k ^ 1;
    e->gbase += n;
    return SG_OK;
}

constexpr int TINY_FALLBACK = 1;
static int tiny_impl(sg_engine* e, const sg_event* ev, const sg_event_ext* ext, uint64_t n, const sg_arg* args,
                     uint64_t n_args, uint32_t* out) {
    if (!e || !ev || !out) return fail(SG_EINVAL, "null argument");
    if (n_args && !args) return fail(SG_EINVAL, "null args table");
    if (!e->fatal.empty()) return fail(SG_ESTATE, e->fatal + " -- engine unusable, recreate it");
    if (n > e->cfg.max_batch_events) return fail(SG_EINVAL, "batch larger than max_batch_events");
    HIPCHK(hipSetDevice(e->device));
    int rc = ensure_batch(e, n);
    if (rc) return rc;
    if ((rc = drain(e))) return rc;
    if ((rc = ensure_pool2(e))) return rc;
    const unsigned long long pfloor = e->h_pool_next ? e->h_pool_next[PC_FLOOR] : 0;
    if (e->pool_nb && e->h_pool_next[PC_NEXT] > pfloor + (e->pool_nb - pfloor) / 2) return TINY_FALLBACK;
    const int k = e->cur;
    activate(e, k);
    auto& B = e->slot[k];
    hipStream_t st = e->stream;
    const sg_event* dev_ev = ev;
    const bool host_out = !is_device_ptr(out);
    if (!is_device_ptr(ev)) {
        HIPCHK(hipMemcpyAsync(e->d_ev, ev, n * sizeof(sg_event), hipMemcpyHostToDevice, st));
        dev_ev = e->d_ev;
    }
    uint32_t* dev_out = host_out ? e->d_out : out;
    const sg_event_ext* dev_ext = ext;
    const sg_arg* dev_args = n_args ? args : nullptr;
    if (ext && !is_device_ptr(ext)) {
        if (n > B.ext_cap) {
            dfree(B.d_ext);
            B.ext_cap = std::max<uint64_t>(n, 1u << 16);
            HIPCHK(hipMalloc(&B.d_ext, B.ext_cap * sizeof(sg_event_ext)));
        }
        HIPCHK(hipMemcpyAsync(B.d_ext, ext, n * sizeof(sg_event_ext), hipMemcpyHostToDevice, st));
        dev_ext = B.d_ext;
    }
    if (n_args && !is_device_ptr(args)) {
        if (n_args > B.args_cap) {
            dfree(B.d_args);
            B.args_cap = std::max<uint64_t>(n_args, 1u << 16);
            HIPCHK(hipMalloc(&B.d_args, B.args_cap * sizeof(sg_arg)));
        }
        HIPCHK(hipMemcpyAsync(B.d_args, args, n_args * sizeof(sg_arg), hipMemcpyHostToDevice, st));
        dev_args = B.d_args;
    }
    if (++e->epoch == 0) e->epoch = 1;
    DevCfg dc;
    std::memset(&dc, 0, sizeof(dc));
    dc.max_rt = e->cfg.statistic_max_rt;
    dc.occupy_timeout = e->cfg.occupy_timeout_ms;
    dc.max_chain = e->cfg.max_slot_chain_size;
    dc.switch_on = e->cfg.switch_on;
    dc.ring_mask = (1ull << e->cfg.status_ring_log2) - 1;
    dc.snap_hi = e->snap_hi;
    dc.dbg_flags = e->dbg_flags;
    dc.heads = e->has_head ? 1u : 0u;
    DevState S{};
    std::memset(&S, 0, sizeof(S));
    S.sec = e->d_sec; S.minb = e->d_minb; S.info = e->d_info; S.prog = e->d_prog; S.rules = e->d_rules;
    S.rstate = e->d_rstate; S.hot = e->d_hot; S.pmap = e->d_pmap; S.pbkt = e->d_pbkt; S.pdat = e->d_pdat;
    S.pbm = e->d_pbm; S.ppre = e->d_ppre; S.tmid = e->d_tmid; S.ring = e->d_ring; S.sink = e->d_sink;
    S.borrow = e->d_borrow; S.prio = e->d_prio; S.key_ring = e->d_keyring; S.gbase = e->gbase; S.link = e->d_link;
    S.bst = e->d_bst; S.pend = e->d_pend; S.spans = e->d_spans; S.nspan = e->d_bsmall + 120; S.span_cap = e->span_cap;
    S.epoch = e->epoch; S.skip_ok = 0; S.skip_min = e->skip_min; S.ext = dev_ext; S.args = dev_args;
    S.aux_tab = e->d_auxtab; S.aux_count = e->d_auxcnt; S.aux_cap = e->cfg.aux_node_capacity; S.aux_mask = e->aux_mask;
    S.max_ctx = SG_MAX_CONTEXTS;
    S.auth = dev_auth(e);
    S.auth_ids = dev_auth_ids(e);
    const int cap = e->cfg.max_slot_chain_size;
    const uint32_t grants = cap <= 0 ? 1u : e->n_chains >= (uint32_t)cap ? 2u : 0u;
    HIPCHK(launch_tiny(dev_ev, (uint32_t)n, S, dc, e->cfg.max_resources, e->d_prio, e->d_comp, n_args, grants,
                       e->d_pool_next, e->pool_nb, e->epoch, e->d_recs, e->d_v0, e->d_dec, e->d_segs, e->d_bsmall,
                       dev_out, st));
    uint32_t bflags = 0;
    HIPCHK(hipMemcpyAsync(&bflags, e->d_bsmall, 4, hipMemcpyDeviceToHost, st));
    if (host_out) HIPCHK(hipMemcpyAsync(out, dev_out, n * 4, hipMemcpyDeviceToHost, st));
    if (e->pool_nb) HIPCHK(hipMemcpyAsync(e->h_pool_next, e->d_pool_next, PC_WORDS * 8, hipMemcpyDeviceToHost, st));
    HIPCHK(hipStreamSynchronize(st));
    if (bflags & BF_TINY_FALLBACK) return TINY_FALLBACK;
    if (bflags & BF_TINY_REJECTED) {
        if (bflags & BF_BAD_RES) return fail(SG_EINVAL, "event res_id >= max_resources");
        if (bflags & BF_BAD_REF)
            return fail(SG_EINVAL, "an EXIT/TRACE references an event that is not an earlier ENTRY of the same resource");
        if (bflags & BF_TSPAN) return fail(SG_EINVAL, "a batch must span less than 2^31 ms");
        if (bflags & BF_BACKWARD) return fail(SG_EINVAL, "event timestamps must be non-decreasing (SURVEY Q3)");
        return fail(SG_EINVAL, "an sg_event_ext names args outside the table (or more than SG_MAX_ARGS, or a bad kind)");
    }
    e->gbase += n;
    if (bflags & BF_BAD_REF)
        return fail(SG_EINVAL, "an EXIT/TRACE references an event that is not an earlier ENTRY of the same resource");
    if (bflags & BF_BACKWARD) return fail(SG_EINVAL, "event timestamps must be non-decreasing across batches (SURVEY Q3)");
    if (bflags & BF_AUX_FULL) return fail(SG_ECAPACITY, "origin/context node pool full (raise aux_node_capacity)");
    if (bflags & BF_PQ_INVARIANT)
        e->fatal = "internal error: a k_pq tile's presorted key subset did not match its accesses";
    else if (bflags & BF_POOL_FULL)
        e->fatal = "the hot-parameter map pool is used up (raise param_table_log2)";
    else if (bflags & BF_PTAB_FULL)
        e->fatal = "a hot-parameter map table could not place a key (its map holds a ghost entry)";
    if (bflags & (BF_PQ_INVARIANT | BF_PTAB_FULL | BF_POOL_FULL)) return fail(SG_ECAPACITY, e->fatal + " -- engine unusable");
    return SG_OK;
}

int sg_submit_async(sg_engine* e, const sg_event* ev, uint64_t n, uint32_t* out) {
    return submit_impl(e, ev, nullptr, n, nullptr, 0, out);
}

int sg_submit_ex_async(sg_engine* e, const sg_event* ev, const sg_event_ext* ext, uint64_t n, const sg_arg* args,
                       uint64_t n_args, uint32_t* out) {
    return submit_impl(e, ev, ext, n, args, n_args, out);
}

int sg_submit_ex(sg_engine* e, const sg_event* ev, const sg_event_ext* ext, uint64_t n, const sg_arg* args,
                 uint64_t n_args, uint32_t* out) {
    if (e && e->tiny_on && n && n <= tiny_max() && !e->radix_group) {
        const int trc = tiny_impl(e, ev, ext, n, args, n_args, out);
        if (trc != TINY_FALLBACK) return trc;
    }
    int rc = submit_impl(e, ev, ext, n, args, n_args, out);
    if (rc) {
        if (e) (void)drain(e);
        return rc;
    }
    return sg_sync(e);
}

int sg_intern_origin(sg_engine* e, const char* origin, uint32_t* out_id) {
    if (!e || !out_id) return fail(SG_EINVAL, "null argument");
    if (!origin || !*origin) { *out_id = 0; return SG_OK; }
    auto it = e->origin_ids.find(origin);
    if (it != e->origin_ids.end()) { *out_id = it->second; return SG_OK; }
    const uint32_t id = (uint32_t)e->origin_ids.size() + 1;
    if (id >= 0x7FFFFFFFu) return fail(SG_ECAPACITY, "too many origins");
    e->origin_ids.emplace(origin, id);
    *out_id = id;
    if (e->auth.by_name.count(origin)) {
        if (int rc = drain(e)) return rc;
        e->auth.on_intern(origin, id);
        if (int rc = upload_authority(e)) return rc;
    }
    if (e->rule_names.count(std::string("o\x01") + origin)) {
        if (int rc = drain(e)) return rc;
        return upload_rules(e, false, false, false);
    }
    return SG_OK;
}

int sg_intern_context(sg_engine* e, const char* context, uint32_t* out_id) {
    if (!e || !out_id) return fail(SG_EINVAL, "null argument");
    if (!context || !*context || !std::strcmp(context, "sentinel_default_context")) { *out_id = 0; return SG_OK; }
    auto it = e->context_ids.find(context);
// ... 468 lines not shown
```

sentinel_amd/csrc/kernels.hip:

```cpp
#include <hip/hip_runtime.h>
#include <stdint.h>
#include <stdlib.h>

#include "../../include/sentinel_gpu.h"
#include "authority.h"
#include "dev_types.h"

using namespace sg;

#define WAVE 64

#define RS_THREADS 256
#ifndef RS_ITEMS
#define RS_ITEMS 16
#endif
#define RS_TILE (RS_THREADS * RS_ITEMS)
#define RS_BINS 256

template <int DB>
__device__ __forceinline__ void hist_add(uint32_t* h, uint32_t d, bool valid) {
    uint64_t peers = __ballot(valid);
#pragma unroll
    for (int b = 0; b < DB; ++b) {
        const uint64_t bb = __ballot((d >> b) & 1);
// ... 957 lines not shown
            sg_metric_node m;
            m.timestamp = b.ws;
            m.pass_qps = b.pass;
            m.block_qps = b.block;
            m.success_qps = b.succ;
            m.exception_qps = b.exc;
            m.rt = b.succ != 0 ? b.rt / b.succ : b.rt;
            m.occupied_pass_qps = b.occ;
            m.res_id = r;
            m.reserved = 0;
            outp[o] = m;
        }
        ++o;
        if (b.ws > nl) nl = b.ws;
    }
    info[r].last_fetch = nl;
}

__global__ void k_init_state(Bkt* __restrict__ sec, Bkt* __restrict__ minb, NodeInfo* __restrict__ info,
                             int64_t* __restrict__ borrow, uint32_t nres) {
    uint64_t i = (uint64_t)blockIdx.x * blockDim.x + threadIdx.x;
    Bkt z;
    z.ws = -1; z.pass = 0; z.block = 0; z.exc = 0; z.succ = 0; z.rt = 0; z.occ = 0; z.minrt = 0;
    if (i < (uint64_t)nres * 60) minb[i] = z;
    if (i < (uint64_t)nres * 2) {
        sec[i] = z;
        borrow[2 * i] = -1;
        borrow[2 * i + 1] = 0;
    }
    if (i < nres) {
        NodeInfo n;
        n.thread = 0; n.flags = 0; n.exc_sum_sec = -1; n.exc_sum = 0; n.last_fetch = -1;
        info[i] = n;
    }
}
__global__ void k_set_flags(NodeInfo* __restrict__ info, const uint64_t* __restrict__ upd, uint32_t n) {
    uint32_t i = blockIdx.x * blockDim.x + threadIdx.x;
    if (i >= n) return;
    uint64_t u = upd[i];
    uint32_t res = (uint32_t)u;
    uint32_t f = (uint32_t)((u >> 32) & 0x7FFFFFFFu);
    if (u >> 63) info[res].flags |= f;
    else info[res].flags &= ~f;
}
__global__ void k_region_copy(const uint64_t* __restrict__ src, uint64_t* __restrict__ dst, const uint64_t* __restrict__ tri) {
    const uint64_t s = tri[3 * blockIdx.x], d = tri[3 * blockIdx.x + 1], n = tri[3 * blockIdx.x + 2];
    for (uint64_t i = threadIdx.x; i < n; i += blockDim.x) dst[d + i] = src[s + i];
}

namespace sg {

hipError_t launch_rs_first(const sg_event* ev, uint64_t n, uint32_t max_res, uint64_t gbase, const uint8_t* ring,
                           uint64_t ring_mask, int32_t max_rt, SEv* rec_o, uint32_t* keys, uint32_t* vals,
                           uint32_t* ghist, uint32_t nblocks, uint32_t* bflags, int64_t* t0_out, uint32_t* prio,
                           uint64_t* key_ring, const uint32_t* comp, const sg_event_ext* ext, const sg_arg* args,
                           uint64_t n_args, uint32_t max_ctx, const AuthDesc* auth, const uint32_t* auth_ids,
                           hipStream_t st) {
    hipLaunchKernelGGL(k_rs_first<8>, dim3(nblocks), dim3(RS_THREADS), 0, st, ev, n, max_res, gbase, ring, ring_mask,
                       max_rt, rec_o, keys, vals, ghist, nblocks, bflags, t0_out, prio, key_ring, comp, ext, args,
                       n_args, max_ctx, auth, auth_ids);
    return hipGetLastError();
}
hipError_t launch_radix_hist(const uint32_t* keys, uint64_t n, int shift, uint32_t* ghist, uint32_t nblocks,
                             hipStream_t st) {
    hipLaunchKernelGGL(k_radix_hist<8>, dim3(nblocks), dim3(RS_THREADS), 0, st, keys, n, shift, ghist, nblocks,
                       (const uint32_t*)nullptr);
    return hipGetLastError();
}
hipError_t launch_radix_hist_n(const uint32_t* keys, uint64_t n, const uint32_t* ndev, int shift, uint32_t* ghist,
                               uint32_t nblocks, hipStream_t st) {
    hipLaunchKernelGGL(k_radix_hist<8>, dim3(nblocks), dim3(RS_THREADS), 0, st, keys, n, shift, ghist, nblocks, ndev);
    return hipGetLastError();
}
hipError_t launch_radix_scatter_n(const uint32_t* kin, const uint32_t* vin, uint64_t n, const uint32_t* ndev, int shift,
                                  const uint32_t* goff, uint32_t nblocks, uint32_t* kout, uint32_t* vout, hipStream_t st) {
    hipLaunchKernelGGL(k_radix_scatter<8>, dim3(nblocks), dim3(RS_THREADS), 0, st, kin, vin, n, shift, goff, nblocks,
                       kout, vout, (uint32_t*)nullptr, ndev, (const uint32_t*)nullptr, (const uint32_t*)nullptr, 0u);
    return hipGetLastError();
}
hipError_t launch_radix_scatter(const uint32_t* kin, const uint32_t* vin, uint64_t n, int shift, const uint32_t* goff,
                                uint32_t nblocks, uint32_t* kout, uint32_t* vout, uint32_t* pos_of, hipStream_t st) {
    hipLaunchKernelGGL(k_radix_scatter<8>, dim3(nblocks), dim3(RS_THREADS), 0, st, kin, vin, n, shift, goff, nblocks,
                       kout, vout, pos_of, (const uint32_t*)nullptr, (const uint32_t*)nullptr, (const uint32_t*)nullptr, 0u);
    return hipGetLastError();
}
hipError_t launch_radix_scatter_x(const uint32_t* kin, const uint32_t* vin, uint64_t n, const uint32_t* ndev,
                                  const uint32_t* tcnt, const uint32_t* dbase, int shift, const uint32_t* goff,
                                  uint32_t nblocks, uint32_t* kout, uint32_t* vout, uint32_t* pos_of, hipStream_t st) {
    hipLaunchKernelGGL(k_radix_scatter<8>, dim3(nblocks), dim3(RS_THREADS), 0, st, kin, vin, n, shift, goff, nblocks,
                       kout, vout, pos_of, ndev, tcnt, dbase, 1u);
    return hipGetLastError();
}
hipError_t launch_grp_first(const sg_event* ev, uint64_t n, uint32_t max_res, uint64_t gbase, uint64_t ring_mask,
                            uint32_t* bflags, int64_t* t0_out, uint32_t* prio, uint64_t* key_ring, const uint32_t* comp,
                            const sg_event_ext* ext, const sg_arg* args, uint64_t n_args, uint32_t max_ctx,
                            const AuthDesc* auth, const uint32_t* auth_ids,
                            const uint16_t* hot_tab, uint32_t nhot, uint32_t nblocks, uint32_t* words,
                            uint32_t* hot_hist, uint32_t* ckeys, uint32_t* cvals, uint32_t* ccnt, uint32_t* chist,
                            hipStream_t st) {
    hipLaunchKernelGGL(k_grp_first<8>, dim3(nblocks), dim3(RS_THREADS), 0, st, ev, n, max_res, gbase, ring_mask, bflags,
                       t0_out, prio, key_ring, comp, ext, args, n_args, max_ctx, auth, auth_ids, hot_tab, nhot, nblocks, words,
                       hot_hist, ckeys, cvals, ccnt, chist);
    return hipGetLastError();
}
hipError_t launch_hot_scan(uint32_t* C, uint32_t nblocks, uint32_t nhot, uint32_t* part, uint32_t* hb, uint32_t* total,
                           hipStream_t st) {
    if (!nhot) return hipMemsetAsync(total, 0, 4, st);
    const uint32_t nch = (nblocks + HS_TC - 1) / HS_TC;
    hipLaunchKernelGGL(k_hot_scan_a, dim3(nch), dim3(256), 0, st, C, nblocks, nhot, part);
    hipLaunchKernelGGL(k_hot_scan_b, dim3(1), dim3(HOT_MAX), 0, st, part, nch, nhot, hb, total);
    hipLaunchKernelGGL(k_hot_scan_c, dim3(nch), dim3(256), 0, st, C, nblocks, nhot, part, hb);
    return hipGetLastError();
}
hipError_t launch_hot_bmax(const sg_event* ev, uint32_t nblocks, const uint32_t* P, uint32_t nhot, const uint32_t* hb,
                           uint32_t* edges, uint32_t* bmax, hipStream_t st) {
    if (!nhot || !nblocks) return hipSuccess;
    hipLaunchKernelGGL(k_bkt_edges, dim3(1), dim3(BE_THREADS), 0, st, ev, nblocks, edges);
    hipLaunchKernelGGL(k_hot_bmax, dim3((nhot + 255) / 256, (nblocks + BM_EDGES - 1) / BM_EDGES), dim3(256), 0, st, P,
                       nblocks, nhot, hb, edges, bmax);
    return hipGetLastError();
}
hipError_t launch_grp_records(const sg_event* ev, uint64_t n, uint64_t gbase, uint64_t ring_mask, int32_t max_rt,
                              const uint32_t* words, const uint32_t* P, uint32_t nhot, uint32_t nblocks,
                              const uint32_t* hb, SEv* recs, uint32_t* svals, uint32_t* prev,
                              uint32_t* nprev, uint32_t* bst, uint32_t* bflags, const sg_event_ext* ext,
                              const sg_arg* args, uint32_t max_ctx, Link* link, uint32_t epoch,
                              const uint32_t* need_hot, const uint32_t* need_blk, hipStream_t st) {
    hipLaunchKernelGGL(k_grp_records, dim3(nblocks * 4), dim3(GR_THREADS), 0, st, ev, n, gbase, ring_mask, max_rt, words, P,
                       nhot, nblocks, hb, recs, svals, prev, nprev, bst, bflags, ext, args, max_ctx, link, epoch, need_hot,
                       need_blk);
    return hipGetLastError();
}
hipError_t launch_hot_segs(const uint32_t* hb, uint32_t nhot, const uint32_t* hot_list, Seg* segs, uint32_t* out,
                           hipStream_t st) {
    hipLaunchKernelGGL(k_hot_segs, dim3(1), dim3(HOT_MAX), 0, st, hb, nhot, hot_list, segs, out);
    return hipGetLastError();
}
hipError_t launch_hot_build(const Seg* segs, const uint32_t* mp, uint32_t mb, uint32_t min_len, uint32_t max_res, uint16_t* hot_tab,
                            uint32_t* hot_list, uint32_t nhot_old, uint32_t* hot_n, hipStream_t st) {
    if (nhot_old) hipLaunchKernelGGL(k_hot_clear, dim3((nhot_old + 255) / 256), dim3(256), 0, st, hot_tab, hot_list, nhot_old);
    if (mb) hipLaunchKernelGGL(k_hot_build, dim3((mb + 255) / 256), dim3(256), 0, st, segs, mp, min_len, max_res, hot_tab,
                               hot_list, hot_n);
    return hipGetLastError();
}
__global__ void k_cold_n(uint64_t n, const uint32_t* __restrict__ hot_total, uint32_t* __restrict__ out) {
    if (threadIdx.x == 0) *out = (uint32_t)(n - *hot_total);
}
hipError_t launch_cold_n(uint64_t n, const uint32_t* hot_total, uint32_t* out, hipStream_t st) {
    hipLaunchKernelGGL(k_cold_n, dim3(1), dim3(64), 0, st, n, hot_total, out);
    return hipGetLastError();
}
uint32_t hot_max() { return HOT_MAX; }

__global__ __launch_bounds__(1024) void k_cold_small(const uint32_t* __restrict__ kin, const uint32_t* __restrict__ vin,
                                                     const uint32_t* __restrict__ cnt_p, const uint32_t* __restrict__ dbase,
                                                     uint32_t* __restrict__ kout, uint32_t* __restrict__ vout,
                                                     uint32_t* __restrict__ words) {
    __shared__ unsigned long long s[RS_TILE];
    const uint32_t cnt = *cnt_p, ob = *dbase, t = threadIdx.x;
    uint32_t n2 = 1;
    while (n2 < cnt) n2 <<= 1;
    for (uint32_t i = t; i < n2; i += blockDim.x)
        s[i] = i < cnt ? (((unsigned long long)kin[i] << 32) | i) : ~0ull;
    __syncthreads();
    for (uint32_t k = 2; k <= n2; k <<= 1)
        for (uint32_t j = k >> 1; j > 0; j >>= 1) {
            for (uint32_t i = t; i < n2; i += blockDim.x) {
                const uint32_t l = i ^ j;
                if (l > i) {
                    const unsigned long long a = s[i], b = s[l];
                    if (((i & k) == 0) == (a > b)) { s[i] = b; s[l] = a; }
                }
            }
            __syncthreads();
        }
    for (uint32_t i = t; i < cnt; i += blockDim.x) {
        const uint32_t idx = (uint32_t)s[i], key = (uint32_t)(s[i] >> 32), v = vin[idx], dst = ob + i;
        kout[dst] = key;
        vout[dst] = v;
        words[v & 0x7FFFFFFFu] = dst | ((v >> 1) & W_ENT);
    }
}
hipError_t launch_cold_small(const uint32_t* kin, const uint32_t* vin, const uint32_t* cnt, const uint32_t* dbase,
                             uint32_t* kout, uint32_t* vout, uint32_t* words, hipStream_t st) {
    hipLaunchKernelGGL(k_cold_small, dim3(1), dim3(1024), 0, st, kin, vin, cnt, dbase, kout, vout, words);
    return hipGetLastError();
}
hipError_t launch_post_w(const uint32_t* words, const uint32_t* P, uint32_t nhot, const uint32_t* dec, uint64_t n,
                         uint64_t gbase, uint8_t* ring, uint64_t ring_mask, uint32_t* out, hipStream_t st) {
    const uint32_t nb = (uint32_t)((n + 256 * POSTW_ITEMS - 1) / (256 * POSTW_ITEMS));
    hipLaunchKernelGGL(k_post_w, dim3(nb), dim3(256), 0, st, words, P, nhot, dec, n, gbase, ring, ring_mask, out);
    return hipGetLastError();
}

uint32_t radix_tile() { return RS_TILE; }

hipError_t launch_init_state(Bkt* sec, Bkt* minb, NodeInfo* info, int64_t* borrow, uint32_t nres, hipStream_t st) {
    uint64_t tot = (uint64_t)nres * 60;
    hipLaunchKernelGGL(k_init_state, dim3((uint32_t)((tot + 255) / 256)), dim3(256), 0, st, sec, minb, info, borrow, nres);
    return hipGetLastError();
}
hipError_t launch_set_flags(NodeInfo* info, const uint64_t* upd, uint32_t n, hipStream_t st) {
    if (!n) return hipSuccess;
    hipLaunchKernelGGL(k_set_flags, dim3((n + 255) / 256), dim3(256), 0, st, info, upd, n);
    return hipGetLastError();
}

hipError_t launch_region_copy(const uint64_t* src, uint64_t* dst, const uint64_t* tri, uint32_t n, hipStream_t st) {
    if (!n) return hipSuccess;
    hipLaunchKernelGGL(k_region_copy, dim3(n), dim3(256), 0, st, src, dst, tri);
    return hipGetLastError();
}

__global__ __launch_bounds__(SC_THREADS) void k_scan_one(const uint32_t* __restrict__ in, uint64_t n,
                                                      uint32_t* __restrict__ out, uint32_t* __restrict__ total) {
    const uint64_t base = (uint64_t)threadIdx.x * SC_ITEMS;
    uint32_t loc[SC_ITEMS];
    uint32_t s = 0;
#pragma unroll
    for (int k = 0; k < SC_ITEMS; ++k) {
        const uint64_t i = base + k;
        loc[k] = i < n ? in[i] : 0;
        s += loc[k];
    }
    uint32_t tot;
    uint32_t ex = block_excl_scan(s, &tot);
#pragma unroll
    for (int k = 0; k < SC_ITEMS; ++k) {
        const uint64_t i = base + k;
        if (i < n) out[i] = ex;
        ex += loc[k];
    }
    if (threadIdx.x == 0 && total) *total = tot;
}
hipError_t launch_scan(const uint32_t* in, uint32_t* out, uint64_t n, uint32_t* part, uint32_t* total,
                       hipStream_t st) {
    if (n <= SC_TILE) {
        hipLaunchKernelGGL(k_scan_one, dim3(1), dim3(SC_THREADS), 0, st, in, n, out, total);
        return hipGetLastError();
    }
    uint32_t nb = (uint32_t)((n + SC_TILE - 1) / SC_TILE);
    if (nb == 0) nb = 1;
    hipLaunchKernelGGL(k_scan_reduce, dim3(nb), dim3(SC_THREADS), 0, st, in, n, part, (const uint32_t*)nullptr);
    hipLaunchKernelGGL(k_scan_top, dim3(1), dim3(SC_THREADS), 0, st, part, nb, total);
    hipLaunchKernelGGL(k_scan_down, dim3(nb), dim3(SC_THREADS), 0, st, in, n, part, out, (const uint32_t*)nullptr);
    return hipGetLastError();
}
hipError_t launch_scan_n(const uint32_t* in, uint32_t* out, uint64_t n, const uint32_t* ndev, uint32_t* part,
                         uint32_t* total, hipStream_t st) {
    uint32_t nb = (uint32_t)((n + SC_TILE - 1) / SC_TILE);
    if (nb == 0) nb = 1;
    hipLaunchKernelGGL(k_scan_reduce, dim3(nb), dim3(SC_THREADS), 0, st, in, n, part, ndev);
    hipLaunchKernelGGL(k_scan_top, dim3(1), dim3(SC_THREADS), 0, st, part, nb, total);
    hipLaunchKernelGGL(k_scan_down, dim3(nb), dim3(SC_THREADS), 0, st, in, n, part, out, ndev);
    return hipGetLastError();
}

hipError_t launch_snapshot(Bkt* minb, NodeInfo* info, uint32_t nres, int64_t now, int32_t max_rt, uint32_t* cnt,
                           uint32_t* off, uint32_t* part, uint32_t* total, sg_metric_node* outp, uint64_t cap,
                           hipStream_t st) {
    uint32_t nb = (nres + 255) / 256;
    hipLaunchKernelGGL(k_snap_count, dim3(nb), dim3(256), 0, st, minb, info, nres, now, max_rt, cnt);
    hipError_t e = launch_scan(cnt, off, nres, part, total, st);
    if (e != hipSuccess) return e;
    hipLaunchKernelGGL(k_snap_emit, dim3(nb), dim3(256), 0, st, minb, info, nres, now, off, outp, cap);
    return hipGetLastError();
}

}
```

sentinel_amd/engine.py:

```python
from __future__ import annotations

import ctypes as C
import os

import numpy as np

from . import _abi as A

_HERE = os.path.dirname(os.path.abspath(__file__))
LIB_PATH = os.environ.get("SG_LIB_PATH") or os.path.join(_HERE, "libsentinel_gpu.so")
_lib = None

EXPORTS = (
    "sg_config_default", "sg_engine_create", "sg_engine_destroy", "sg_register_resources", "sg_resource_id",
    "sg_load_flow_rules", "sg_load_degrade_rules", "sg_load_param_rules", "sg_param_key", "sg_submit",
    "sg_submit_async", "sg_sync", "sg_snapshot_metrics", "sg_cluster_set_connected_count",
    "sg_cluster_request_tokens", "sg_cluster_request_param_tokens", "sg_read_node", "sg_last_error", "sg_last_timings",
    "sg_submit_ex", "sg_submit_ex_async", "sg_intern_origin", "sg_intern_context", "sg_param_thread_count",
    "sg_cluster_namespace", "sg_cluster_assign_flows", "sg_cluster_set_namespace_connected",
    "sg_cluster_namespace_qps", "sg_load_authority_rules", "sg_param_intern", "sg_param_intern_batch",
    "sg_param_keys_sweep", "sg_param_keys_stats",
)


# ... 71 lines not shown

    def __init__(self, **cfg):
        self._cfg = default_config(**cfg)
        h = C.c_void_p()
        _check(lib().sg_engine_create(C.byref(self._cfg), C.byref(h)))
        self.h = h
        self.n_events = 0

    def close(self):
        if getattr(self, "h", None):
            lib().sg_engine_destroy(self.h)
            self.h = None

    def __del__(self):
        try:
            self.close()
        except Exception:
            pass

    def register(self, name: str) -> int:
        return self.register_many([name])[0]

    def register_many(self, names) -> np.ndarray:
        arr = (C.c_char_p * max(1, len(names)))(*[n.encode() if isinstance(n, str) else n for n in names])
        out = np.zeros(len(names), dtype=np.uint32)
        _check(lib().sg_register_resources(self.h, arr, len(names), out.ctypes.data_as(C.POINTER(C.c_uint32))))
        return out

    def register_ptrs(self, names_ptr, n: int):
        _check(lib().sg_register_resources(self.h, C.cast(names_ptr, C.POINTER(C.c_char_p)), n, None))

    def resource_id(self, name: str) -> int:
        out = C.c_uint32()
        _check(lib().sg_resource_id(self.h, name.encode(), C.byref(out)))
        return out.value

    def _load(self, fn, rules, struct):
        if isinstance(rules, tuple):
            ptr, n = rules
        else:
            arr = (struct * max(1, len(rules)))(*rules)
            ptr, n = C.cast(arr, C.c_void_p), len(rules)
        out = C.c_uint32()
        _check(fn(self.h, ptr, n, C.byref(out)))
        return out.value

    def load_flow_rules(self, rules) -> int:
        return self._load(lib().sg_load_flow_rules, rules, A.SgFlowRule)

    def load_degrade_rules(self, rules) -> int:
        return self._load(lib().sg_load_degrade_rules, rules, A.SgDegradeRule)

    def load_param_rules(self, rules) -> int:
        return self._load(lib().sg_load_param_rules, rules, A.SgParamRule)

    def load_authority_rules(self, rules) -> int:
        return self._load(lib().sg_load_authority_rules, rules, A.SgAuthorityRule)

    def param_intern(self, value, class_type="java.lang.String") -> int:
        out = C.c_uint64()
        _check(lib().sg_param_intern(self.h, None if value is None else str(value).encode(),
                                     None if class_type is None else class_type.encode(), C.byref(out)))
        return out.value

    def param_intern_many(self, values, class_types="java.lang.String") -> np.ndarray:
        n = len(values)
        enc = [v if v is None or isinstance(v, bytes) else str(v).encode() for v in values]
        vals = (C.c_char_p * max(1, n))(*enc)
        if class_types is None or isinstance(class_types, str):
            ct = None if class_types is None else class_types.encode()
            types = (C.c_char_p * max(1, n))(*([ct] * n))
        else:
            types = (C.c_char_p * max(1, n))(*[None if t is None else t.encode() for t in class_types])
        out = np.zeros(n, dtype=np.uint64)
        _check(lib().sg_param_intern_batch(self.h, vals, types, n, out.ctypes.data_as(C.POINTER(C.c_uint64))))
        return out

    def param_keys_sweep(self) -> dict:
        _check(lib().sg_param_keys_sweep(self.h))
        return self.param_keys_stats()

    def param_keys_stats(self) -> dict:
        out = (C.c_uint64 * 8)()
        k = lib().sg_param_keys_stats(self.h, out, 8)
        names = ("entries", "displaced", "pinned", "sweeps", "candidates", "held", "dropped", "sweep_us")
        return {names[i]: int(out[i]) for i in range(k)}

    def keysweep_scans(self):
        fn = lib().sgx_keysweep_scans
        fn.restype = C.c_int
        fn.argtypes = [C.c_void_p, C.POINTER(C.c_double)]
        out = (C.c_double * 3)()
        if fn(self.h, out) != 0:
            raise SentinelError(A.SG_EDEVICE, "sgx_keysweep_scans failed")
        return tuple(out)

    def submit(self, events: np.ndarray) -> np.ndarray:
        ev = np.ascontiguousarray(events, dtype=A.EVENT_DTYPE)
        out = np.zeros(len(ev), dtype=np.uint32)
        _check(lib().sg_submit(self.h, ev.ctypes.data, len(ev), out.ctypes.data))
        self.n_events += len(ev)
        return out

    def submit_ex(self, events: np.ndarray, ext: np.ndarray = None, args: np.ndarray = None) -> np.ndarray:
        ev = np.ascontiguousarray(events, dtype=A.EVENT_DTYPE)
        ex = None if ext is None else np.ascontiguousarray(ext, dtype=A.EXT_DTYPE)
        ar = None if args is None or len(args) == 0 else np.ascontiguousarray(args, dtype=A.ARG_DTYPE)
        out = np.zeros(len(ev), dtype=np.uint32)
        _check(lib().sg_submit_ex(self.h, ev.ctypes.data, None if ex is None else ex.ctypes.data, len(ev),
                                  None if ar is None else ar.ctypes.data, 0 if ar is None else len(ar), out.ctypes.data))
        self.n_events += len(ev)
        return out

    def intern_origin(self, name: str) -> int:
        out = C.c_uint32()
        _check(lib().sg_intern_origin(self.h, name.encode(), C.byref(out)))
        return out.value

    def intern_context(self, name: str) -> int:
        out = C.c_uint32()
        _check(lib().sg_intern_context(self.h, name.encode(), C.byref(out)))
        return out.value

    def submit_ptr(self, ev_ptr: int, n: int, out_ptr: int, sync: bool = True):
        if sync:
            _check(lib().sg_submit(self.h, C.c_void_p(ev_ptr), n, C.c_void_p(out_ptr)))
        else:
            _check(lib().sg_submit_async(self.h, C.c_void_p(ev_ptr), n, C.c_void_p(out_ptr)))
        self.n_events += n

    def submit_ex_ptr(self, ev_ptr: int, ext_ptr: int, n: int, out_ptr: int, sync: bool = True, args_ptr: int = 0,
                      n_args: int = 0):
        fn = lib().sg_submit_ex if sync else lib().sg_submit_ex_async
        _check(fn(self.h, C.c_void_p(ev_ptr), C.c_void_p(ext_ptr) if ext_ptr else None, n,
                  C.c_void_p(args_ptr) if args_ptr else None, n_args, C.c_void_p(out_ptr)))
        self.n_events += n

    def sync(self):
        _check(lib().sg_sync(self.h))

    def timings(self):
        ms = (C.c_double * 4)()
        k = lib().sg_last_timings(self.h, ms, 4)
        return list(ms[:k])

    def timing_log(self, cap: int = 4096) -> np.ndarray:
        buf = (C.c_double * (4 * cap))()
        fn = lib().sgx_timing_log
        fn.restype = C.c_int
        fn.argtypes = [C.c_void_p, C.c_void_p, C.c_int]
        k = fn(self.h, buf, cap)
        return np.frombuffer(buf, dtype=np.float64, count=4 * k).reshape(k, 4).copy()

    def spans_total(self) -> int:
        fn = lib().sgx_spans_total
        fn.restype = C.c_ulonglong
        fn.argtypes = [C.c_void_p]
        return int(fn(self.h))

    def hot_marked(self) -> int:
        fn = lib().sgx_hot_marked
        fn.restype = C.c_uint
        fn.argtypes = [C.c_void_p]
        return int(fn(self.h))

    def read_aux_node(self, res: int, kind: int, node_id: int):
        fn = lib().sgx_read_aux_node
        fn.restype = C.c_int
        fn.argtypes = [C.c_void_p, C.c_uint32, C.c_uint32, C.c_uint32, C.c_void_p]
        out = np.zeros(21, dtype=np.int64)
        rc = fn(self.h, res, kind, node_id, out.ctypes.data)
        if rc < 0:
            raise SentinelError(A.SG_EDEVICE, "sgx_read_aux_node failed")
        if rc == 0:
            return None
        return {"second": out[:16].reshape(2, 8), "thread": int(out[16]), "mhist": out[17:21].reshape(2, 2)}

    def pv_last(self) -> dict:
        fn = lib().sgx_pv_last
        fn.restype = C.c_int
        fn.argtypes = [C.c_void_p, C.c_void_p]
        out = np.zeros(7, dtype=np.uint64)
        if fn(self.h, out.ctypes.data) != 0:
            raise SentinelError(A.SG_EDEVICE, "sgx_pv_last failed")
        return {"segments": int(out[0]), "accesses": int(out[1]), "ranges": int(out[2]),
                "post_segments": int(out[3]), "post_ops": int(out[4]), "post_done": int(out[5]),
                "walk_max": int(out[6])}

    def param_pool(self) -> dict:
        fn = lib().sgx_param_pool
        fn.restype = C.c_int
        fn.argtypes = [C.c_void_p, C.c_void_p]
        out = np.zeros(5, dtype=np.uint64)
        if fn(self.h, out.ctypes.data) != 0:
            raise SentinelError(A.SG_EDEVICE, "sgx_param_pool failed")
        return {"buckets": int(out[0]), "taken": int(out[1]), "floor": int(out[2]), "compactions": int(out[3]),
                "device_compactions": int(out[4])}

    def param_compact(self):
        fn = lib().sgx_param_compact
        fn.restype = C.c_int
        fn.argtypes = [C.c_void_p]
        if fn(self.h) != 0:
            raise SentinelError(A.SG_EDEVICE, "sgx_param_compact failed")

    def param_thread_count(self, res: int, idx: int, key: int, with_presence: bool = False):
        fn = lib().sg_param_thread_count
        fn.restype = C.c_int
        fn.argtypes = [C.c_void_p, C.c_uint32, C.c_int32, C.c_uint64, C.POINTER(C.c_int64), C.POINTER(C.c_int32)]
        c, p = C.c_int64(), C.c_int32()
        _check(fn(self.h, res, idx, key, C.byref(c), C.byref(p)))
        return (c.value, bool(p.value)) if with_presence else c.value

    def read_node(self, res: int, now: int = 0) -> dict:
        st = A.SgNodeState()
        _check(lib().sg_read_node(self.h, res, now, C.byref(st)))
        return A.node_state_to_numpy(st)

    def snapshot(self, now: int, cap: int = 1 << 16) -> np.ndarray:
        out = np.zeros(cap, dtype=A.METRIC_NODE_DTYPE)
        n = C.c_uint64()
        _check(lib().sg_snapshot_metrics(self.h, int(now), out.ctypes.data, cap, C.byref(n)))
        return out[: min(cap, n.value)]

    def snapshot_to(self, now: int, out_ptr: int, cap: int) -> int:
        n = C.c_uint64()
        _check(lib().sg_snapshot_metrics(self.h, int(now), C.c_void_p(out_ptr), cap, C.byref(n)))
        return n.value

    def cluster_set_connected(self, flow_id: int, n: int):
        _check(lib().sg_cluster_set_connected_count(self.h, int(flow_id), int(n)))

    def cluster_namespace(self, name, max_qps: float) -> int:
        out = C.c_uint32()
        _check(lib().sg_cluster_namespace(self.h, None if name is None else str(name).encode(), float(max_qps),
                                          C.byref(out)))
        return out.value

    def cluster_assign_flows(self, name: str, flow_ids):
        ids = np.ascontiguousarray(flow_ids, dtype=np.int64).reshape(-1)
        _check(lib().sg_cluster_assign_flows(self.h, name.encode(), ids.ctypes.data_as(C.POINTER(C.c_int64)), len(ids)))

    def cluster_set_namespace_connected(self, name: str, n: int):
        _check(lib().sg_cluster_set_namespace_connected(self.h, name.encode(), int(n)))

    def cluster_namespace_qps(self, name: str, now: int):
        cur, lim = C.c_double(), C.c_double()
        _check(lib().sg_cluster_namespace_qps(self.h, name.encode(), int(now), C.byref(cur), C.byref(lim)))
        return cur.value, lim.value

    def cluster_request_array(self, reqs: np.ndarray) -> np.ndarray:
        reqs = np.ascontiguousarray(reqs, dtype=A.TOKEN_REQ_DTYPE)
        out = np.zeros(len(reqs), dtype=A.TOKEN_RES_DTYPE)
        _check(lib().sg_cluster_request_tokens(self.h, reqs.ctypes.data, len(reqs), out.ctypes.data))
        return out

    def cluster_request_ptr(self, req_ptr: int, n: int, out_ptr: int):
        _check(lib().sg_cluster_request_tokens(self.h, C.c_void_p(req_ptr), n, C.c_void_p(out_ptr)))

    def cluster_request(self, reqs):
        arr = np.zeros(len(reqs), dtype=A.TOKEN_REQ_DTYPE)
        for i, (ts, fid, acq, pr) in enumerate(reqs):
            arr[i] = (ts, fid, acq, int(pr))
        out = self.cluster_request_array(arr)
        return [(int(o["status"]), int(o["remaining"]), int(o["wait_in_ms"])) for o in out]

    def cluster_request_param_array(self, reqs: np.ndarray, values: np.ndarray) -> np.ndarray:
        reqs = np.ascontiguousarray(reqs, dtype=A.PARAM_TOKEN_REQ_DTYPE)
        values = np.ascontiguousarray(values, dtype=np.uint64)
        out = np.zeros(len(reqs), dtype=A.TOKEN_RES_DTYPE)
        _check(lib().sg_cluster_request_param_tokens(self.h, reqs.ctypes.data, len(reqs), values.ctypes.data,
                                                     len(values), out.ctypes.data))
        return out

    def cluster_request_param(self, reqs):
        arr, vals = A.param_token_arrays(reqs)
        out = self.cluster_request_param_array(arr, vals)
        return [(int(o["status"]), int(o["remaining"]), int(o["wait_in_ms"])) for o in out]
```

Measured before the change: 4.531 billion.

## Defer decide-stage enqueue to overlap next batch grouping with previous decide

Splits submit into a group stage and a deferred decide stage, so the host no longer blocks on the grouping stream before returning. The decide work for batch N is now enqueued after batch N+1's first grouping kernel has been launched. Event sets rotate through a ring of four and batch headers and flags are read through pinned host buffers, replacing synchronous memcpys. Three memsets are fused into one clear kernel. The cost is much more complex error handling, held errors, and deferred state, which could introduce ordering bugs.

```diff
diff --git a/sentinel_amd/csrc/engine.cpp b/sentinel_amd/csrc/engine.cpp
--- a/sentinel_amd/csrc/engine.cpp
+++ b/sentinel_amd/csrc/engine.cpp
@@ -8,6 +8,7 @@
 #include <cstdio>
 #include <cstdlib>
 #include <cstring>
+#include <deque>
 #include <functional>
 #include <map>
 #include <set>
@@ -62,6 +63,8 @@
 hipError_t launch_cold_small(const uint32_t* kin, const uint32_t* vin, const uint32_t* cnt, const uint32_t* dbase,
                              uint32_t* kout, uint32_t* vout, uint32_t* words, hipStream_t st);
 uint32_t hot_max();
+hipError_t launch_grp_clear(uint32_t* bsmall, uint32_t nsmall, uint32_t* bst, uint32_t nbst, uint32_t* need,
+                            uint32_t nneed, hipStream_t st);
 hipError_t launch_seg_cold(const uint32_t* keys, uint64_t n, const uint32_t* lo, const uint32_t* sbase, uint32_t* flag,
                            uint32_t* pos, Seg* segs, hipStream_t st,
                            hipError_t (*scan)(const uint32_t*, uint32_t*, uint64_t, uint32_t*, uint32_t*, hipStream_t),
@@ -536,13 +539,35 @@
         Link* d_link = nullptr;
         uint32_t *d_bst = nullptr, *d_pend = nullptr;
         Span* d_spans = nullptr;
-        hipEvent_t ev[5] = {nullptr, nullptr, nullptr, nullptr, nullptr};
-        bool pending = false;
+        hipEvent_t* ev = nullptr;
+        hipEvent_t last_post = nullptr;
+        uint32_t* h_head = nullptr;
+        struct Grouped {
+            uint64_t n = 0, n_args = 0, gbase = 0, ring_mask = 0;
+            const sg_event* dev_ev = nullptr;
+            const sg_event_ext* dev_ext = nullptr;
+            const sg_arg* dev_args = nullptr;
+            uint32_t *out = nullptr, *dev_out = nullptr, *vin = nullptr;
+            uint32_t epoch = 0, skip_min = 0, lane_max = 0, mb = 0;
+            bool ext = false, host_out = false, force_lane = false;
+            int set = 0;
+        } g;
     } slot[2];
     int cur = 0;
     int last = -1;
+    int grouped = -1;
+    int held_rc = 0;
+    std::string held_msg;
+    bool handoff_late = true;
+    static constexpr int N_SETS = 4;
+    hipEvent_t evset[N_SETS][5] = {};
+    uint32_t* h_mirror = nullptr;
+    uint64_t seq = 0;
+    struct InFlight { int set; uint32_t hot_marked; };
+    std::deque<InFlight> inflight;
     hipStream_t gstream = nullptr;
     std::vector<std::array<double, 4>> tlog;
+    std::vector<std::array<double, 2>> glog;
     std::string fatal;
     uint32_t* d_prio = nullptr;
     uint16_t* d_hot_tab = nullptr;
@@ -679,6 +704,8 @@
     uint64_t snap_cap = 0;
 };
 
+static int handoff(sg_engine* e);
+
 namespace {
 
 constexpr uint64_t SHARD_BATCH = 3ull << 21;
@@ -763,26 +790,37 @@
     return SG_OK;
 }
 
-static int collect(sg_engine* e, int k) {
-    auto& B = e->slot[k];
-    if (!B.pending) return SG_OK;
-    B.pending = false;
-    HIPCHK(hipEventSynchronize(B.ev[4]));
+constexpr uint32_t HEAD_WORDS = 77;
+constexpr uint32_t MIRROR_WORDS = 121;
+
+static int collect(sg_engine* e) {
+    if (e->inflight.empty()) return SG_OK;
+    const sg_engine::InFlight f = e->inflight.front();
+    e->inflight.pop_front();
+    hipEvent_t* ev = e->evset[f.set];
+    HIPCHK(hipEventSynchronize(ev[4]));
     float g = 0, d = 0, p = 0;
-    (void)hipEventElapsedTime(&g, B.ev[0], B.ev[1]);
-    (void)hipEventElapsedTime(&d, B.ev[2], B.ev[3]);
-    (void)hipEventElapsedTime(&p, B.ev[3], B.ev[4]);
+    (void)hipEventElapsedTime(&g, ev[0], ev[1]);
+    (void)hipEventElapsedTime(&d, ev[2], ev[3]);
+    (void)hipEventElapsedTime(&p, ev[3], ev[4]);
     (void)hipGetLastError();
     e->last_ms[0] = g; e->last_ms[1] = d; e->last_ms[2] = p; e->last_ms[3] = (double)g + d + p;
     e->tlog.push_back({(double)g, (double)d, (double)p, (double)g + d + p});
     if (e->tlog.size() > 4096) e->tlog.erase(e->tlog.begin(), e->tlog.begin() + 2048);
-    uint32_t bflags = 0;
-    HIPCHK(hipMemcpyAsync(&bflags, B.d_bsmall, 4, hipMemcpyDeviceToHost, e->gstream));
-    uint32_t nspan = 0;
-    HIPCHK(hipMemcpyAsync(&nspan, B.d_bsmall + 120, 4, hipMemcpyDeviceToHost, e->gstream));
-    HIPCHK(hipStreamSynchronize(e->gstream));
-    e->spans_total += nspan;
-    e->hot_marked_last = B.hot_marked;
+    float ga = 0, gb = 0;
+    const uint64_t collected = e->seq - e->inflight.size() - 1;
+    if (collected > 0) {
+        hipEvent_t* pv = e->evset[(f.set + sg_engine::N_SETS - 1) % sg_engine::N_SETS];
+        if (hipEventElapsedTime(&ga, pv[1], ev[0]) != hipSuccess) ga = NAN;
+        if (hipEventElapsedTime(&gb, pv[4], ev[2]) != hipSuccess) gb = NAN;
+        (void)hipGetLastError();
+    }
+    e->glog.push_back({(double)ga, (double)gb});
+    if (e->glog.size() > 4096) e->glog.erase(e->glog.begin(), e->glog.begin() + 2048);
+    const uint32_t* mir = e->h_mirror + (size_t)f.set * MIRROR_WORDS;
+    const uint32_t bflags = mir[0];
+    e->spans_total += mir[120];
+    e->hot_marked_last = f.hot_marked;
     if (bflags & BF_BAD_REF)
         return fail(SG_EINVAL, "an EXIT/TRACE references an event that is not an earlier ENTRY of the same resource");
     if (bflags & BF_BACKWARD)
@@ -803,13 +841,20 @@
 static inline const uint32_t* dev_auth_ids(const sg_engine* e) { return e->auth_on ? e->d_auth_ids : nullptr; }
 
 static int drain(sg_engine* e) {
-    int rc = SG_OK;
-    for (int i = 0; i < 2; ++i) {
-        int r = collect(e, (e->cur + i) & 1);
-        if (r && !rc) rc = r;
-    }
+    int rc = e->held_rc;
+    std::string msg = e->held_msg;
+    e->held_rc = 0;
+    auto note = [&](int r) {
+        if (r && !rc) { rc = r; msg = g_err; }
+    };
+    note(handoff(e));
+    while (!e->inflight.empty()) note(collect(e));
     HIPCHK(hipStreamSynchronize(e->stream));
-    return rc;
+    return rc ? fail(rc, msg) : SG_OK;
+}
+static void drain_hold(sg_engine* e) {
+    const int rc = drain(e);
+    if (rc) { e->held_rc = rc; e->held_msg = g_err; }
 }
 
 
@@ -1200,8 +1245,15 @@
     if (hipStreamCreateWithPriority(&e->gstream, hipStreamNonBlocking, prio_lo) != hipSuccess) {
         return bad(fail(SG_EDEVICE, "stream"));
     }
-    for (auto& B : e->slot)
-        for (auto& v : B.ev) if (hipEventCreate(&v) != hipSuccess) return bad(fail(SG_EDEVICE, "event"));
+    for (auto& s : e->evset)
+        for (auto& v : s) if (hipEventCreate(&v) != hipSuccess) return bad(fail(SG_EDEVICE, "event"));
+    for (auto& B : e->slot) {
+        if (hipHostMalloc(&B.h_head, HEAD_WORDS * 4) != hipSuccess) return bad(fail(SG_ENOMEM, "pinned batch head"));
+        B.ev = e->evset[0];
+    }
+    if (hipHostMalloc(&e->h_mirror, sg_engine::N_SETS * MIRROR_WORDS * 4) != hipSuccess)
+        return bad(fail(SG_ENOMEM, "pinned batch flags"));
+    std::memset(e->h_mirror, 0, sg_engine::N_SETS * MIRROR_WORDS * 4);
     uint64_t R = cfg.max_resources;
     if (hipMalloc(&e->d_sec, R * 2 * sizeof(Bkt)) != hipSuccess || hipMalloc(&e->d_minb, R * 60 * sizeof(Bkt)) != hipSuccess ||
         hipMalloc(&e->d_info, R * sizeof(NodeInfo)) != hipSuccess || hipMalloc(&e->d_prog, R * sizeof(Prog)) != hipSuccess ||
@@ -1247,6 +1299,7 @@
     if (const char* v = std::getenv("SG_HEAD_MIN")) e->head_min = (uint32_t)std::strtoul(v, nullptr, 0);
     if (const char* v = std::getenv("SG_J4_MAX")) { e->j4_max = (uint32_t)std::strtoul(v, nullptr, 0); e->bins_pinned = true; }
     if (const char* v = std::getenv("SG_PIPELINE")) e->pipeline = v[0] == '1';
+    if (const char* v = std::getenv("SG_HANDOFF")) e->handoff_late = v[0] != '0';
     if (const char* v = std::getenv("SG_TINY")) e->tiny_on = v[0] != '0';
     if (const char* v = std::getenv("SG_LITE_CHECK")) { if (v[0] == '1') e->dbg_flags |= LITE_CHECK; }
     if (const char* v = std::getenv("SG_RADIX_BELOW")) e->radix_below = std::strtoull(v, nullptr, 0);
@@ -1276,26 +1329,35 @@
 
 extern "C" int sgx_timing_log(sg_engine* e, double* out, int cap) {
     if (!e || !out) return 0;
-    (void)drain(e);
+    drain_hold(e);
     int k = 0;
     for (; k < cap && k < (int)e->tlog.size(); ++k)
         for (int j = 0; j < 4; ++j) out[4 * k + j] = e->tlog[k][j];
     e->tlog.clear();
     return k;
 }
+extern "C" int sgx_gap_log(sg_engine* e, double* out, int cap) {
+    if (!e || !out) return 0;
+    drain_hold(e);
+    int k = 0;
+    for (; k < cap && k < (int)e->glog.size(); ++k)
+        for (int j = 0; j < 2; ++j) out[2 * k + j] = e->glog[k][j];
+    e->glog.clear();
+    return k;
+}
 extern "C" unsigned long long sgx_spans_total(sg_engine* e) {
     if (!e) return 0;
-    (void)drain(e);
+    drain_hold(e);
     return e->spans_total;
 }
 extern "C" unsigned int sgx_hot_marked(sg_engine* e) {
     if (!e) return 0;
-    (void)drain(e);
+    drain_hold(e);
     return e->hot_marked_last;
 }
 extern "C" int sgx_debug_reset(sg_engine* e) {
     if (!e || !e->d_dbg) return 0;
-    (void)drain(e);
+    drain_hold(e);
     unsigned long long z[64] = {0};
     z[20] = ~0ull;
     return hipMemcpy(e->d_dbg, z, sizeof(z), hipMemcpyHostToDevice) == hipSuccess ? 1 : 0;
@@ -1373,6 +1435,7 @@
 int sg_engine_destroy(sg_engine* e) {
     if (!e) return SG_OK;
     (void)hipSetDevice(e->device);
+    e->grouped = -1;
     if (e->stream) (void)hipStreamSynchronize(e->stream);
     if (e->gstream) (void)hipStreamSynchronize(e->gstream);
     dfree(e->d_sec); dfree(e->d_minb); dfree(e->d_info); dfree(e->d_prog); dfree(e->d_rules); dfree(e->d_rstate);
@@ -1391,8 +1454,10 @@
     dfree(e->d_snap_cnt); dfree(e->d_snap_off); dfree(e->d_snap_out); dfree(e->d_dbg);
     dfree(e->d_ks_key); dfree(e->d_ks_idx); dfree(e->d_ks_marks);
     for (auto& v : e->ks_ev) if (v) (void)hipEventDestroy(v);
-    for (auto& B : e->slot)
-        for (auto& v : B.ev) if (v) (void)hipEventDestroy(v);
+    for (auto& s : e->evset)
+        for (auto& v : s) if (v) (void)hipEventDestroy(v);
+    for (auto& B : e->slot) if (B.h_head) (void)hipHostFree(B.h_head);
+    if (e->h_mirror) (void)hipHostFree(e->h_mirror);
     if (e->gstream) (void)hipStreamDestroy(e->gstream);
     for (auto& v : e->join) if (v) (void)hipEventDestroy(v);
     if (e->fork) (void)hipEventDestroy(e->fork);
@@ -2289,29 +2354,15 @@
     return a.type == hipMemoryTypeDevice || a.type == hipMemoryTypeManaged;
 }
 
-static int submit_impl(sg_engine* e, const sg_event* ev, const sg_event_ext* ext, uint64_t n, const sg_arg* args,
-                       uint64_t n_args, uint32_t* out) {
-    if (!e || (n && (!ev || !out))) return fail(SG_EINVAL, "null argument");
-    if (n_args && !args) return fail(SG_EINVAL, "null args table");
-    if (!e->fatal.empty()) return fail(SG_ESTATE, e->fatal + " -- engine unusable, recreate it");
-    if (n == 0) return SG_OK;
-    if (n > e->cfg.max_batch_events || n >= (1ull << 31)) return fail(SG_EINVAL, "batch larger than max_batch_events");
-    HIPCHK(hipSetDevice(e->device));
-    int rc = ensure_batch(e, n);
-    if (rc) return rc;
-    const int k = e->cur;
-    rc = collect(e, k);
-    if (rc) return rc;
-    if (int prc = ensure_pool2(e)) return prc;
-    const unsigned long long pfloor = e->h_pool_next ? e->h_pool_next[PC_FLOOR] : 0;
-    if (e->pool_nb && e->h_pool_next[PC_NEXT] > pfloor + (e->pool_nb - pfloor) / 2) {
-        if (int drc = drain(e)) return drc;
-        if (int crc = compact_pmaps(e)) return crc;
-        ++e->n_compact;
-    }
+static int decide_stage(sg_engine* e, int k);
+
+static int group_stage(sg_engine* e, int k, const sg_event* ev, const sg_event_ext* ext, uint64_t n, const sg_arg* args,
+                       uint64_t n_args, uint32_t* out, int* prev) {
     activate(e, k);
     auto& B = e->slot[k];
-    hipStream_t gs = e->gstream, st = e->stream;
+    B.ev = e->evset[e->seq % sg_engine::N_SETS];
+    hipStream_t gs = e->gstream;
+    if (B.last_post) HIPCHK(hipStreamWaitEvent(gs, B.last_post, 0));
     const sg_event* dev_ev = ev;
     bool host_in = !is_device_ptr(ev);
     bool host_out = !is_device_ptr(out);
@@ -2341,8 +2392,8 @@
         dev_args = B.d_args;
     }
     const uint64_t ring_mask = (1ull << e->cfg.status_ring_log2) - 1;
-    if (!e->pipeline && e->last >= 0 && e->slot[e->last].pending)
-        HIPCHK(hipStreamWaitEvent(gs, e->slot[e->last].ev[4], 0));
+    if (!e->pipeline && e->last >= 0 && e->slot[e->last].last_post)
+        HIPCHK(hipStreamWaitEvent(gs, e->slot[e->last].last_post, 0));
     HIPCHK(hipEventRecord(B.ev[0], gs));
     uint32_t R = e->cfg.max_resources;
     int bits = 1;
@@ -2350,11 +2401,12 @@
     const int db = 8;
     int passes = (bits + db - 1) / db;
     uint32_t nblocks = (uint32_t)((n + radix_tile() - 1) / radix_tile());
-    HIPCHK(hipMemsetAsync(e->d_bsmall, 0, 256 * 4, gs));
     int64_t* d_t0 = reinterpret_cast<int64_t*>(e->d_bsmall + 4);
     uint32_t *kin = e->d_k1, *vin = e->d_v1, *kout = e->d_k0, *vout = e->d_v0;
     if (++e->epoch == 0) e->epoch = 1;
     B.radix = e->radix_group || n >= (1ull << 30) || n < e->radix_below;
+    HIPCHK(launch_grp_clear(e->d_bsmall, 256, e->d_bst, B.radix ? 0u : (uint32_t)((n + 1023) / 1024), e->d_need,
+                            B.radix ? 0u : (uint32_t)e->need_words, gs));
     const bool force_lane = !e->cfg.switch_on || (e->dbg_flags & 2);
     const uint32_t mb = (uint32_t)std::min<uint64_t>(n, R);
     const uint32_t nblk = (mb + 255) / 256;
@@ -2384,10 +2436,19 @@
         HIPCHK(launch_seg_order(e->d_segs, e->d_bsmall + 1, mb, e->d_blkcnt, e->d_order, e->d_bsmall + 8, gs));
         return SG_OK;
     };
+    auto decide_prev = [&]() -> int {
+        if (*prev < 0) return SG_OK;
+        const int pk = *prev;
+        *prev = -1;
+        const int drc = decide_stage(e, pk);
+        activate(e, k);
+        return drc;
+    };
     if (B.radix) {
         HIPCHK(launch_rs_first(dev_ev, n, R, e->gbase, e->d_ring, ring_mask, e->cfg.statistic_max_rt, e->d_rec_o,
                                e->d_k1, e->d_v1, e->d_hist, nblocks, e->d_bsmall + 0, d_t0, e->d_prio, e->d_keyring,
                                e->d_comp, dev_ext, dev_args, n_args, SG_MAX_CONTEXTS, dev_auth(e), dev_auth_ids(e), gs));
+        if (int drc = decide_prev()) return drc;
         for (int p = 0; p < passes; ++p) {
             if (p > 0) HIPCHK(launch_radix_hist(kin, n, p * db, e->d_hist, nblocks, gs));
             HIPCHK(launch_scan(e->d_hist, e->d_hist, (uint64_t)nblocks << db, e->d_part, nullptr, gs));
@@ -2410,6 +2471,7 @@
                                 e->d_comp, dev_ext, dev_args, n_args, SG_MAX_CONTEXTS, dev_auth(e), dev_auth_ids(e),
                                 e->d_hot_tab, nhot, nblocks,
                                 words, hot_off, e->d_k1, e->d_v1, ccnt, e->d_hist, gs));
+        if (int drc = decide_prev()) return drc;
         HIPCHK(launch_hot_scan(hot_off, nblocks, nhot, e->d_hot_part, e->d_hot_hb, e->d_bsmall + 77, gs));
         HIPCHK(launch_cold_n(n, e->d_bsmall + 77, e->d_bsmall + 78, gs));
         if (nblocks == 1) {
@@ -2431,13 +2493,11 @@
         const uint64_t sc = nblocks + 64;
         HIPCHK(launch_seg_cold(kin, n, e->d_bsmall + 77, e->d_bsmall + 80, ccnt + sc, ccnt + 2 * sc, e->d_segs, gs,
                                launch_scan, e->d_part, e->d_bsmall + 82, e->d_bsmall + 1));
-        HIPCHK(hipMemsetAsync(e->d_bst, 0, ((n + 1023) / 1024) * 4, gs));
         uint32_t *need_hot = nullptr, *need_blk = nullptr, *bmax = nullptr;
         if (!(e->dbg_flags & TABLES_ALL)) {
             need_hot = e->d_need;
             need_blk = e->d_need + hot_max();
             bmax = e->d_need + e->need_words - hot_max();
-            HIPCHK(hipMemsetAsync(e->d_need, 0, e->need_words * 4, gs));
             HIPCHK(launch_hot_bmax(dev_ev, nblocks, hot_off, nhot, e->d_hot_hb, e->d_edges, bmax, gs));
         }
         if (int brc = bins(need_hot, need_blk, bmax)) return brc;
@@ -2452,18 +2512,30 @@
     if (!B.radix)
         HIPCHK(launch_hot_build(e->d_segs, e->d_bsmall + 1, mb, hot_min, R, e->d_hot_tab, e->d_hot_list, e->nhot,
                                 e->d_bsmall + 76, gs));
-    uint32_t head[77];
-    static_assert(8 + N_BINS + 1 <= 72, "head layout");
-    HIPCHK(hipMemcpyAsync(head, e->d_bsmall, sizeof(head), hipMemcpyDeviceToHost, gs));
+    static_assert(8 + N_BINS + 1 <= 72 && HEAD_WORDS == 77, "head layout");
+    HIPCHK(hipMemcpyAsync(B.h_head, e->d_bsmall, HEAD_WORDS * 4, hipMemcpyDeviceToHost, gs));
     HIPCHK(hipEventRecord(B.ev[1], gs));
-    HIPCHK(hipStreamSynchronize(gs));
+    auto& G = B.g;
+    G.n = n; G.n_args = n_args; G.gbase = e->gbase; G.ring_mask = ring_mask;
+    G.dev_ev = dev_ev; G.dev_ext = dev_ext; G.dev_args = dev_args;
+    G.out = out; G.dev_out = dev_out; G.vin = vin;
+    G.epoch = e->epoch; G.skip_min = skip_min; G.lane_max = lane_max; G.mb = mb;
+    G.ext = ext != nullptr; G.host_out = host_out; G.force_lane = force_lane;
+    G.set = (int)(e->seq % sg_engine::N_SETS);
+    e->grouped = k;
+    return SG_OK;
+}
+
+static int accept_grouped(sg_engine* e, bool drop = false) {
+    const int k = e->grouped;
+    auto& B = e->slot[k];
+    e->grouped = -1;
+    HIPCHK(hipEventSynchronize(B.ev[1]));
+    const uint32_t* head = B.h_head;
     if (!B.radix) e->nhot = std::min<uint32_t>(head[76], hot_max());
+    if (drop) return SG_OK;
     B.hot_marked = head[73];
-    const uint32_t m = head[1];
-    const uint32_t nprev = head[3];
-    int64_t t0 = 0;
-    std::memcpy(&t0, head + 4, 8);
-    uint32_t bflags = head[0];
+    const uint32_t bflags = head[0];
     if (bflags & BF_BAD_RES) return fail(SG_EINVAL, "event res_id >= max_resources");
     if (bflags & BF_BAD_REF)
         return fail(SG_EINVAL, "an EXIT/TRACE references an event that is not an earlier ENTRY of the same resource");
@@ -2471,6 +2543,56 @@
     if (bflags & BF_BACKWARD) return fail(SG_EINVAL, "event timestamps must be non-decreasing (SURVEY Q3)");
     if (bflags & BF_BAD_ARGS)
         return fail(SG_EINVAL, "an sg_event_ext names args outside the table (or more than SG_MAX_ARGS, or a bad kind)");
+    if (e->has_mix && head[7] && (e->pv_on || e->pvt_on) && head[72]) {
+        if (int prc = ensure_pv(e, head[72], head[7])) return prc;
+    }
+    e->inflight.push_back({B.g.set, B.hot_marked});
+    ++e->seq;
+    e->last = k;
+    e->cur = k ^ 1;
+    e->gbase += B.g.n;
+    return SG_OK;
+}
+
+static int handoff(sg_engine* e) {
+    if (e->grouped < 0) return SG_OK;
+    const int k = e->grouped;
+    if (int rc = accept_grouped(e)) return rc;
+    return decide_stage(e, k);
+}
+
+static int decide_enqueue(sg_engine* e, int k);
+
+static int decide_stage(sg_engine* e, int k) {
+    const int rc = decide_enqueue(e, k);
+    if (rc) {
+        const std::string why = g_err;
+        if (!e->inflight.empty()) e->inflight.pop_back();
+        if (e->fatal.empty()) e->fatal = "the decide stage of an accepted batch could not be enqueued (" + why + ")";
+        return fail(rc, why);
+    }
+    return rc;
+}
+
+static int decide_enqueue(sg_engine* e, int k) {
+    activate(e, k);
+    auto& B = e->slot[k];
+    const auto& G = B.g;
+    hipStream_t st = e->stream;
+    const uint64_t n = G.n, n_args = G.n_args, ring_mask = G.ring_mask;
+    const sg_event* dev_ev = G.dev_ev;
+    const sg_event_ext* dev_ext = G.dev_ext;
+    const sg_arg* dev_args = G.dev_args;
+    uint32_t *out = G.out, *dev_out = G.dev_out, *vin = G.vin;
+    const uint32_t skip_min = G.skip_min, lane_max = G.lane_max, mb = G.mb;
+    const bool ext = G.ext, host_out = G.host_out, force_lane = G.force_lane;
+    (void)n_args;
+    const uint32_t* head = B.h_head;
+    const uint32_t m = head[1];
+    const uint32_t nprev = head[3];
+    int64_t t0 = 0;
+    std::memcpy(&t0, head + 4, 8);
+    const uint32_t bflags = head[0];
     const uint32_t* off = head + 8;
     uint32_t bin_n[N_BINS];
     for (int b = 0; b < N_BINS; ++b) bin_n[b] = off[b + 1] - off[b];
@@ -2504,14 +2626,14 @@
     S.borrow = e->d_borrow;
     S.prio = e->d_prio;
     S.key_ring = e->d_keyring;
-    S.gbase = e->gbase;
+    S.gbase = G.gbase;
     S.link = e->d_link;
     S.bst = e->d_bst;
     S.pend = e->d_pend;
     S.spans = e->d_spans;
     S.nspan = e->d_bsmall + 120;
     S.span_cap = e->span_cap;
-    S.epoch = e->epoch;
+    S.epoch = G.epoch;
     S.skip_ok = !(bflags & (BF_MULTI_LINK | BF_ZERO_CNT)) && !(e->dbg_flags & 4) ? 1u : 0u;
     S.skip_min = skip_min;
     S.ext = dev_ext;
@@ -2586,7 +2708,7 @@
         const uint32_t nm = (uint32_t)e->pmap_key.size();
         HIPCHK(launch_pm_grow(e->d_segs, e->d_bsmall + 1, mb, Sg, e->d_pool_next, e->pool_nb, e->d_bsmall + 0, e->d_pmoves,
                               e->d_pmoves ? reinterpret_cast<uint32_t*>(e->d_pmoves + e->pmoves_cap) : nullptr,
-                              (uint32_t)e->pmoves_cap, e->epoch, nm, e->d_pbkt2, e->d_pdat2, e->d_pcwork,
+                              (uint32_t)e->pmoves_cap, G.epoch, nm, e->d_pbkt2, e->d_pdat2, e->d_pcwork,
                               e->d_pcwork + e->pmoves_cap, e->d_pcwork + 2 * e->pmoves_cap, launch_scan, st));
         HIPCHK(hipMemcpyAsync(e->h_pool_next, e->d_pool_next, PC_WORDS * 8, hipMemcpyDeviceToHost, st));
     }
@@ -2707,14 +2829,65 @@
                           B.d_amulti, S, dc, t0, e->d_dec, e->d_auxpool, e->auxpool_cap, e->d_bsmall + 134, e->d_auxmeta,
                           e->d_bsmall + 0, st));
     HIPCHK(hipEventRecord(B.ev[3], st));
-    if (B.radix) HIPCHK(launch_post(e->d_posof, e->d_dec, n, e->gbase, e->d_ring, ring_mask, dev_out, st));
-    else HIPCHK(launch_post_w(e->d_flag, e->d_pos, B.nhot, e->d_dec, n, e->gbase, e->d_ring, ring_mask, dev_out, st));
+    if (B.radix) HIPCHK(launch_post(e->d_posof, e->d_dec, n, G.gbase, e->d_ring, ring_mask, dev_out, st));
+    else HIPCHK(launch_post_w(e->d_flag, e->d_pos, B.nhot, e->d_dec, n, G.gbase, e->d_ring, ring_mask, dev_out, st));
     if (host_out) HIPCHK(hipMemcpyAsync(out, dev_out, n * 4, hipMemcpyDeviceToHost, st));
+    HIPCHK(hipMemcpyAsync(e->h_mirror + (size_t)G.set * MIRROR_WORDS, e->d_bsmall, MIRROR_WORDS * 4, hipMemcpyDeviceToHost,
+                          st));
     HIPCHK(hipEventRecord(B.ev[4], st));
-    B.pending = true;
-    e->last = k;
-    e->cur = k ^ 1;
-    e->gbase += n;
+    B.last_post = B.ev[4];
+    return SG_OK;
+}
+
+static int submit_impl(sg_engine* e, const sg_event* ev, const sg_event_ext* ext, uint64_t n, const sg_arg* args,
+                       uint64_t n_args, uint32_t* out) {
+    if (!e || (n && (!ev || !out))) return fail(SG_EINVAL, "null argument");
+    if (n_args && !args) return fail(SG_EINVAL, "null args table");
+    if (!e->fatal.empty()) return fail(SG_ESTATE, e->fatal + " -- engine unusable, recreate it");
+    if (n == 0) return SG_OK;
+    if (n > e->cfg.max_batch_events || n >= (1ull << 31)) return fail(SG_EINVAL, "batch larger than max_batch_events");
+    HIPCHK(hipSetDevice(e->device));
+    if (e->held_rc) return drain(e);
+    const bool late = e->handoff_late && e->pipeline && e->cfg.max_slot_chain_size <= 0;
+    int rc;
+    if (n > e->cap_n && (rc = drain(e))) return rc;
+    if ((rc = ensure_batch(e, n))) return rc;
+    if ((rc = ensure_pool2(e))) return rc;
+    int prev = e->grouped;
+    if (prev >= 0 && (rc = accept_grouped(e))) return rc;
+    auto give_up = [&](int why) -> int {
+        if (prev >= 0) {
+            const std::string msg = g_err;
+            const int pk = prev;
+            prev = -1;
+            if (decide_stage(e, pk) == SG_OK) g_err = msg;
+        }
+        return why;
+    };
+    const unsigned long long pfloor = e->h_pool_next ? e->h_pool_next[PC_FLOOR] : 0;
+    const bool compact = e->pool_nb && e->h_pool_next[PC_NEXT] > pfloor + (e->pool_nb - pfloor) / 2;
+    if (!late || compact) {
+        if (prev >= 0) {
+            const int pk = prev;
+            prev = -1;
+            if ((rc = decide_stage(e, pk))) return rc;
+        }
+        while (e->inflight.size() > 1)
+            if ((rc = collect(e))) return rc;
+    }
+    if (compact) {
+        if (int drc = drain(e)) return drc;
+        if (int crc = compact_pmaps(e)) return crc;
+        ++e->n_compact;
+    }
+    const int k = e->cur;
+    if ((rc = group_stage(e, k, ev, ext, n, args, n_args, out, &prev))) return give_up(rc);
+    if (!late) return handoff(e);
+    while (e->inflight.size() > 1)
+        if ((rc = collect(e))) {
+            (void)accept_grouped(e, true);
+            return rc;
+        }
     return SG_OK;
 }
 
diff --git a/sentinel_amd/csrc/kernels.hip b/sentinel_amd/csrc/kernels.hip
--- a/sentinel_amd/csrc/kernels.hip
+++ b/sentinel_amd/csrc/kernels.hip
@@ -1133,6 +1133,21 @@
 }
 uint32_t hot_max() { return HOT_MAX; }
 
+__global__ void k_grp_clear(uint32_t* __restrict__ bsmall, uint32_t nsmall, uint32_t* __restrict__ bst, uint32_t nbst,
+                            uint32_t* __restrict__ need, uint32_t nneed) {
+    const uint32_t i = blockIdx.x * blockDim.x + threadIdx.x;
+    if (i < nsmall) bsmall[i] = 0;
+    if (i < nbst) bst[i] = 0;
+    if (i < nneed) need[i] = 0;
+}
+hipError_t launch_grp_clear(uint32_t* bsmall, uint32_t nsmall, uint32_t* bst, uint32_t nbst, uint32_t* need,
+                            uint32_t nneed, hipStream_t st) {
+    uint32_t m = nsmall > nbst ? nsmall : nbst;
+    if (nneed > m) m = nneed;
+    hipLaunchKernelGGL(k_grp_clear, dim3((m + 255) / 256), dim3(256), 0, st, bsmall, nsmall, bst, nbst, need, nneed);
+    return hipGetLastError();
+}
+
 __global__ __launch_bounds__(1024) void k_cold_small(const uint32_t* __restrict__ kin, const uint32_t* __restrict__ vin,
                                                      const uint32_t* __restrict__ cnt_p, const uint32_t* __restrict__ dbase,
                                                      uint32_t* __restrict__ kout, uint32_t* __restrict__ vout,
diff --git a/sentinel_amd/engine.py b/sentinel_amd/engine.py
--- a/sentinel_amd/engine.py
+++ b/sentinel_amd/engine.py
@@ -247,6 +247,14 @@
         k = fn(self.h, buf, cap)
         return np.frombuffer(buf, dtype=np.float64, count=4 * k).reshape(k, 4).copy()
 
+    def gap_log(self, cap: int = 4096) -> np.ndarray:
+        buf = (C.c_double * (2 * cap))()
+        fn = lib().sgx_gap_log
+        fn.restype = C.c_int
+        fn.argtypes = [C.c_void_p, C.c_void_p, C.c_int]
+        k = fn(self.h, buf, cap)
+        return np.frombuffer(buf, dtype=np.float64, count=2 * k).reshape(k, 2).copy()
+
     def spans_total(self) -> int:
         fn = lib().sgx_spans_total
         fn.restype = C.c_ulonglong
```

New measurement: 4.697 billion (median of 6 runs). 3.7% higher.
